# Mrhs121/distributed

Measured on AMD Instinct MI355X. Metric: images/sec (whole node) MNIST CNN at 1/2/4/8 MI355X; DP scaling efficiency, higher is better.
Workload: dtype bf16; 1 GPU; model=MNIST CNN (Conv2D32-3x3-relu, MaxPool2, Dense64-relu, Dense10; 347,146 params), global_batch=64, per_gpu_batch=64, parallelism=dp1, engine=fused_convnet, optimizer=SGD(lr=1e-3), fp32 master weights

## Files before the change

### csrc/bindings.cpp

```cpp
#include <pybind11/pybind11.h>
#include <pybind11/stl.h>

#include <stdexcept>
#include <string>
#include <unordered_map>
#include <vector>

#include "comm.h"
#include "convnet.h"
#include "damd_common.h"
#include "kernels_api.h"
#include "peer_comm.h"
#include "step_executor.h"

namespace py = pybind11;
using namespace damd;

#define HIP_CHECK(x)                                                                    \
  do {                                                                                  \
    hipError_t e_ = (x);                                                                \
    if (e_ != hipSuccess)                                                               \
      throw std::runtime_error(std::string("HIP error: ") + hipGetErrorString(e_) +     \
                               " at " #x);                                              \
  } while (0)

template <typename T>
static T* P_(uintptr_t p) { return reinterpret_cast<T*>(p); }

class ConvNetTrainer : public StepExecutor {
 public:
  ConvNetTrainer(int device, py::dict bufs, int B, int PP, int grad_allreduce)
      : StepExecutor(device), B_(B), PP_(PP), grad_allreduce_(grad_allreduce) {
    if (B <= 0) throw std::invalid_argument("batch must be > 0");
    if (B > 65535) throw std::invalid_argument("per-rank batch must be < 65536 (packed kernel argument)");
    if (PP < 1 || PP > 4) throw std::invalid_argument("positions per slice must be in [1,4]");
    auto g = [&](const char* k) -> uintptr_t { return bufs[k].cast<uintptr_t>(); };
    b_.X = nullptr; b_.labels = nullptr; b_.x_u8 = 0;
    b_.P = P_<float>(g("params")); b_.G = P_<float>(g("grads")); b_.V = P_<float>(g("velocity"));
    b_.ctrl = P_<Ctrl>(g("ctrl"));
    b_.pooled = P_<uint16_t>(g("pooled")); b_.code = P_<uint8_t>(g("code"));
    b_.W1alt = P_<float>(g("w1alt")); b_.V1alt = P_<float>(g("v1alt")); b_.w1bf = P_<uint16_t>(g("w1bf"));
    b_.stamps = bufs.contains("stamps") ? P_<unsigned long long>(g("stamps")) : nullptr;
    b_.eager_w1 = bufs.contains("eager_w1") ? (int)g("eager_w1") : 0;
    b_.hacc = P_<long long>(g("hacc"));
    b_.hconv = P_<long long>(g("hconv"));
    b_.calt = P_<float>(g("calt"));
    b_.ppb = bufs.contains("ppb") ? (int)g("ppb") : PP;
    b_.force_generic = bufs.contains("specialised") ? !(int)g("specialised") : 0;
    b_.xnext = bufs.contains("xnext") ? P_<void>(g("xnext")) : nullptr;
    b_.xtag = bufs.contains("xtag") ? P_<long long>(g("xtag")) : nullptr;
    b_.xcur = bufs.contains("xcur") ? P_<void>(g("xcur")) : nullptr;
    b_.ycur = bufs.contains("ycur") ? P_<int>(g("ycur")) : nullptr;
    if ((b_.xnext == nullptr) != (b_.xtag == nullptr) || (b_.xcur == nullptr) != (b_.ycur == nullptr))
      throw std::invalid_argument("xnext / xtag and xcur / ycur go in pairs");
    const char* ph = getenv("DAMD_PAR_HINT");
    hint_ = !(ph && ph[0] == '0');
    b_.par_hint = -1;
    if (b_.ppb < 1 || b_.ppb > 4) throw std::invalid_argument("bwd positions per slice must be in [1,4]");
    HIP_CHECK(convnet2_set_lds_limits());
  }
  std::vector<std::vector<float>> phase_times(int k) {
    if (!b_.X) throw std::runtime_error("ConvNetTrainer: set_data() not called");
    hipEvent_t ev[4];
    for (auto& e : ev) HIP_CHECK(hipEventCreate(&e));
    std::vector<std::vector<float>> out;
    for (int i = 0; i < k; ++i) {
      HIP_CHECK(hipEventRecord(ev[0], stream_));
      b_.par_hint = hint_ ? par_ : -1;
      HIP_CHECK(convnet2_launch_fwd(b_, B_, PP_, stream_));
      HIP_CHECK(hipEventRecord(ev[1], stream_));
      HIP_CHECK(convnet2_launch_bwd(b_, B_, PP_, stream_));
      par_ ^= 1;
      HIP_CHECK(hipEventRecord(ev[2], stream_));
      if (grad_allreduce_ && !sharded_) {
        if (peer_ && fold_)
          peer_->allreduce_staged((long)convnet_grad_count(PP_), 2 * kConvNetNConv, stream_, b_.hconv);
        else if (peer_) peer_->allreduce(b_.G, (long)convnet_grad_count(PP_), stream_, b_.hconv, 2 * kConvNetNConv);
        else if (comm_) comm_->allreduce_f32_i64(b_.G, convnet_grad_count(PP_), b_.hconv, 2 * kConvNetNConv, stream_);
      }
      HIP_CHECK(hipEventRecord(ev[3], stream_));
      HIP_CHECK(hipEventSynchronize(ev[3]));
      std::vector<float> r(3);
      for (int j = 0; j < 3; ++j) HIP_CHECK(hipEventElapsedTime(&r[j], ev[j], ev[j + 1]));
      out.push_back(r);
    }
    for (auto& e : ev) hipEventDestroy(e);
    return out;
  }
  void set_data(uintptr_t X, uintptr_t labels, int x_u8) {
    b_.X = P_<const void>(X); b_.labels = P_<const int>(labels); b_.x_u8 = x_u8;
    if (b_.xtag) HIP_CHECK(hipMemsetAsync(b_.xtag, 0, sizeof(long long), stream_));
    invalidate_graphs();
  }
  void set_peer_fold(PeerAllreduce* p, bool fold) {
    if (!G_own_) { G_own_ = b_.G; hconv_own_ = b_.hconv; }
    set_peer(p);
    fold_ = fold && p && p->world() > 1;
    if (fold_) {
      const long n = (long)convnet_grad_count(PP_), nfp = (n + 3) / 4 * 4;
      if (PeerAllreduce::message_words(n, 2 * kConvNetNConv) > p->capacity())
        throw std::invalid_argument("peer all-reduce capacity too small for the folded step");
      b_.G = p->in_local();
      b_.hconv = hconv_own_;
      b_.Gr = p->out_local();
      b_.hconv_r = reinterpret_cast<long long*>(p->out_local() + nfp);
    } else {
      b_.G = G_own_; b_.hconv = hconv_own_; b_.Gr = nullptr; b_.hconv_r = nullptr;
    }
    invalidate_graphs();
  }
  bool folded() const { return fold_; }
  void set_sharded(PeerAllreduce* p, uintptr_t hred, int gbf16) {
    if (!p || p->world() < 2 || p->world() > kXMaxRanks) throw std::invalid_argument("sharded step: 2..8 ranks");
    const int NU = 4 * convnet_num_slices(b_.ppb);
    if (p->capacity() < convnet_xin_floats(p->world(), NU) || p->capacity() < convnet_xout_floats(NU))
      throw std::invalid_argument("sharded step: peer staging too small");
    const PeerArgs& a = p->args();
    XArgs x{};
    for (int r = 0; r < p->world(); ++r) {
      if (!a.in[r] || !a.out[r]) throw std::runtime_error("sharded step: peer staging not mapped");
      x.in[r] = a.in[r];
      x.out[r] = a.out[r];
    }
    x.status = a.status;
    x.timeout_ticks = a.timeout_ticks;
    x.world = p->world();
    x.rank = p->rank();
    x.gbf16 = gbf16;
    x.ppb = b_.ppb;
    xa_ = x;
    set_peer(p);
    sharded_ = true;
    fold_ = false;
    HIP_CHECK(hipMemset(p->out_local() + kXFlags, 0,
                        (size_t)(convnet_xout_floats(NU) - kXFlags) * sizeof(float)));
    HIP_CHECK(hipDeviceSynchronize());
    b_.xa = &xa_;
    b_.Gr = p->out_local() + kXGred;
    b_.hconv_r = P_<long long>(hred);
    invalidate_graphs();
  }
  bool sharded() const { return sharded_; }
  void set_exchange_timeout(double s) { xa_.timeout_ticks = (unsigned long long)(s * 1e8); invalidate_graphs(); }
  void gather() {
    if (sharded_) HIP_CHECK(convnet2_launch_gather(b_, PP_, stream_));
  }
  std::vector<float> metric_tail() {
    std::vector<float> t(3);
    gather();
    HIP_CHECK(hipStreamSynchronize(stream_));
    const float* g = b_.Gr ? b_.Gr : b_.G;
    HIP_CHECK(hipMemcpy(t.data(), g + kConvNetNParam, 3 * sizeof(float), hipMemcpyDeviceToHost));
    return t;
  }
  void flush() {
    gather();
    HIP_CHECK(convnet2_launch_flush(b_, B_, stream_));
    par_ = 0;
  }
  int parity() const { return par_; }
  void capture_final(int k) { StepExecutor::capture_final(k); }
  bool run_final(int k) { return StepExecutor::run_final(k); }
  bool warm_final(int k) { return StepExecutor::warm_final(k); }
  int num_slices() const { return convnet_num_slices(PP_); }
  int num_slices_bwd() const { return convnet_num_slices(b_.ppb); }
  int batch() const { return B_; }
  std::string step_kernels() const { return convnet2_specialised(b_, B_, PP_) ? "specialised" : "generic"; }
  int fwd_threads() const { return convnet2_fwd_threads(b_, B_, PP_); }
  int fwd_compiled_threads() const {
    int n = 0;
    HIP_CHECK(convnet2_fwd_compiled_threads(b_, B_, PP_, &n));
    return n;
  }
  int bwd_threads() const { return convnet2_bwd_threads(b_, B_, PP_); }
  int bwd_compiled_threads() const {
    int n = 0;
    HIP_CHECK(convnet2_bwd_compiled_threads(b_, B_, PP_, &n));
    return n;
  }

 protected:
  void enqueue_tail() override { flush(); }
  int phase_value() const override { return par_; }
  void set_phase(int p) override { par_ = p; }
  int phase_after(int p, int k, bool tail) const override { return tail ? 0 : p ^ (k & 1); }
  void enqueue_one_step() override {
    if (!b_.X) throw std::runtime_error("ConvNetTrainer: set_data() not called");
    b_.par_hint = hint_ ? par_ : -1;
    HIP_CHECK(convnet2_launch_step(b_, B_, PP_, stream_));
    par_ ^= 1;
    if (!grad_allreduce_ || sharded_) return;
    long long* aux = b_.hconv;
    const long n64 = 2 * kConvNetNConv;
    if (peer_ && fold_)
      peer_->allreduce_staged((long)convnet_grad_count(PP_), n64, stream_, b_.hconv);
    else if (peer_)
      peer_->allreduce(b_.G, (long)convnet_grad_count(PP_), stream_, aux, n64);
    else if (comm_)
      comm_->allreduce_f32_i64(b_.G, convnet_grad_count(PP_), aux, (size_t)n64, stream_);
  }

 private:
  ConvNetBuffers b_{};
  float* G_own_ = nullptr;
  long long* hconv_own_ = nullptr;
  bool fold_ = false;
  bool sharded_ = false;
  XArgs xa_{};
  int par_ = 0;
  bool hint_ = true;
  int B_, PP_, grad_allreduce_;
};

const char* damd_src_hash();

PYBIND11_MODULE(_C, m) {
  m.doc() = "distributed_amd native runtime (HIP/gfx950 kernels, RCCL, hipGraph executor)";
  m.def("src_hash", []() { return std::string(damd_src_hash()); });
  m.def("graph_nodes", [](uintptr_t gp) {
    hipGraph_t g = reinterpret_cast<hipGraph_t>(gp);
    size_t n = 0;
    HIP_CHECK(hipGraphGetNodes(g, nullptr, &n));
    std::vector<hipGraphNode_t> nodes(n);
    if (n) HIP_CHECK(hipGraphGetNodes(g, nodes.data(), &n));
    std::unordered_map<hipGraphNode_t, int> idx;
    for (size_t i = 0; i < n; ++i) idx[nodes[i]] = (int)i;
    py::list out;
    for (size_t i = 0; i < n; ++i) {
      hipGraphNodeType t;
      HIP_CHECK(hipGraphNodeGetType(nodes[i], &t));
      std::string name;
      if (t == hipGraphNodeTypeKernel) {
        hipKernelNodeParams kp{};
        if (hipGraphKernelNodeGetParams(nodes[i], &kp) == hipSuccess && kp.func) {
          const char* nm = hipKernelNameRefByPtr(kp.func, nullptr);
          if (nm) name = nm;
        }
        (void)hipGetLastError();
      }
      size_t nd = 0;
      HIP_CHECK(hipGraphNodeGetDependencies(nodes[i], nullptr, &nd));
      std::vector<hipGraphNode_t> deps(nd);
      if (nd) HIP_CHECK(hipGraphNodeGetDependencies(nodes[i], deps.data(), &nd));
      std::vector<int> di;
      for (auto d : deps) di.push_back(idx.count(d) ? idx[d] : -1);
      out.append(py::make_tuple((int)t, name, di));
    }
    return out;
  });
  m.attr("CONVNET_NPARAM") = kConvNetNParam;
  m.attr("CONVNET_NGRAD") = kConvNetNGrad;
  m.attr("CONVNET_NCONV") = kConvNetNConv;
  m.def("convnet2_lds_bytes", [](int PP) { return py::make_tuple(convnet2_fwd_lds(PP, 4), convnet2_bwd_lds(PP)); });
  m.def("convnet2_bwd_flag_lds_bytes", [](int PP) { return convnet2_bwd_lds(PP, true); });
  m.def("convnet_num_slices", &convnet_num_slices);
  m.def("convnet_hacc_elems", &convnet_hacc_elems);
  m.def("convnet_grad_count", &convnet_grad_count);

  m.def("device_count", []() { int n = 0; if (hipGetDeviceCount(&n) != hipSuccess) n = 0; return n; });
  m.def("rccl_unique_id", []() { return py::bytes(rccl_unique_id()); });
  m.def("rccl_version", []() { int v = 0; ncclGetVersion(&v); return v; });

  py::class_<RcclComm>(m, "RcclComm")
      .def(py::init([](int n, int r, py::bytes uid, int dev) {
             return new RcclComm(n, r, std::string(uid), dev);
           }),
           py::arg("nranks"), py::arg("rank"), py::arg("uid"), py::arg("device"),
           py::call_guard<py::gil_scoped_release>())
      .def_property_readonly("nranks", &RcclComm::nranks)
      .def_property_readonly("rank", &RcclComm::rank)
      .def_property_readonly("comm_count", &RcclComm::comm_count)
      .def("allreduce",
           [](RcclComm& c, uintptr_t s, uintptr_t r, size_t n, int dt, int op, uintptr_t st) {
             c.allreduce(P_<void>(s), P_<void>(r), n, dt, op, P_<ihipStream_t>(st));
           })
      .def("broadcast",
           [](RcclComm& c, uintptr_t b, size_t n, int dt, int root, uintptr_t st) {
             c.broadcast(P_<void>(b), n, dt, root, P_<ihipStream_t>(st));
           })
      .def("allgather",
           [](RcclComm& c, uintptr_t s, uintptr_t r, size_t n, int dt, uintptr_t st) {
             c.allgather(P_<const void>(s), P_<void>(r), n, dt, P_<ihipStream_t>(st));
           })
      .def("reduce_scatter",
           [](RcclComm& c, uintptr_t s, uintptr_t r, size_t n, int dt, int op, uintptr_t st) {
             c.reduce_scatter(P_<const void>(s), P_<void>(r), n, dt, op, P_<ihipStream_t>(st));
           })
      .def("allreduce_f32_i64",
           [](RcclComm& c, uintptr_t d, size_t n, uintptr_t a, size_t n64, uintptr_t st) {
             c.allreduce_f32_i64(P_<float>(d), n, P_<long long>(a), n64, P_<ihipStream_t>(st));
           })
      .def("abort", &RcclComm::abort)
      .def_property_readonly("aborted", &RcclComm::aborted);

  m.def("stream_wait", [](uintptr_t st, double timeout_s) {
    py::gil_scoped_release nogil;
    return stream_wait_with_deadline(P_<ihipStream_t>(st), timeout_s, nullptr);
  });

  py::class_<PeerAllreduce>(m, "PeerAllreduce")
      .def(py::init<int, int, int, long, int, double>(), py::arg("world"), py::arg("rank"), py::arg("device"),
           py::arg("capacity"), py::arg("blocks") = 64, py::arg("timeout_s") = 120.0)
      .def("handles", [](PeerAllreduce& p) { return py::bytes(p.handles()); })
      .def("open",
           [](PeerAllreduce& p, std::vector<py::bytes> hs) {
             std::vector<std::string> v;
             for (auto& h : hs) v.emplace_back(std::string(h));
             p.open(v);
           })
      .def("allreduce",
           [](PeerAllreduce& p, uintptr_t data, long n, uintptr_t st, uintptr_t aux64, long n64) {
             p.allreduce(P_<float>(data), n, P_<ihipStream_t>(st), P_<long long>(aux64), n64);
           },
           py::arg("data"), py::arg("n"), py::arg("stream"), py::arg("aux64") = 0, py::arg("n64") = 0)
      .def_static("message_words", &PeerAllreduce::message_words)
      .def("link_local", &PeerAllreduce::link_local)
      .def("status", &PeerAllreduce::status)
      .def("clear_status", &PeerAllreduce::clear_status)
      .def("set_timeout", &PeerAllreduce::set_timeout)
      .def_property_readonly("ready", &PeerAllreduce::ready)
      .def_property_readonly("capacity", &PeerAllreduce::capacity)
      .def("peek_out",
           [](PeerAllreduce& p, long off, long n) {
             std::vector<uint32_t> v((size_t)n);
             HIP_CHECK(hipDeviceSynchronize());
             HIP_CHECK(hipMemcpy(v.data(), p.out_local() + off, (size_t)n * 4, hipMemcpyDeviceToHost));
             return v;
           })
      .def_property_readonly("world", &PeerAllreduce::world)
      .def_property_readonly("rank", &PeerAllreduce::rank);

  py::class_<ConvNetTrainer>(m, "ConvNetTrainer")
      .def(py::init<int, py::dict, int, int, int>(), py::arg("device"), py::arg("buffers"),
           py::arg("batch"), py::arg("positions_per_slice") = 4, py::arg("grad_allreduce") = 1)
      .def("set_data", &ConvNetTrainer::set_data, py::arg("x"), py::arg("labels"), py::arg("x_u8") = 0)
      .def("set_comm", [](ConvNetTrainer& t, RcclComm* c) { t.set_comm(c); },
           py::keep_alive<1, 2>())
      .def("set_peer", [](ConvNetTrainer& t, PeerAllreduce* p, bool fold) { t.set_peer_fold(p, fold); },
           py::arg("peer"), py::arg("fold") = false, py::keep_alive<1, 2>())
      .def_property_readonly("folded", &ConvNetTrainer::folded)
      .def("set_sharded", &ConvNetTrainer::set_sharded, py::arg("peer"), py::arg("hred"), py::arg("gbf16") = 0,
           py::keep_alive<1, 2>())
      .def_property_readonly("sharded", &ConvNetTrainer::sharded)
      .def("set_exchange_timeout", &ConvNetTrainer::set_exchange_timeout)
      .def("gather", &ConvNetTrainer::gather)
      .def("restrict_cus", &ConvNetTrainer::restrict_cus, py::arg("part"), py::arg("nparts"))
      .def("metric_tail", &ConvNetTrainer::metric_tail)
      .def("step", &ConvNetTrainer::step, py::call_guard<py::gil_scoped_release>())
      .def("capture", &ConvNetTrainer::capture)
      .def("step_graph_nodes", &ConvNetTrainer::step_graph_nodes, py::arg("steps"))
      .def("run", &ConvNetTrainer::run, py::call_guard<py::gil_scoped_release>())
      .def("capture_final", &ConvNetTrainer::capture_final, py::arg("steps"))
      .def("run_final", &ConvNetTrainer::run_final, py::arg("steps"), py::call_guard<py::gil_scoped_release>())
      .def("warm_final", &ConvNetTrainer::warm_final, py::arg("steps"), py::call_guard<py::gil_scoped_release>())
      .def("phase_times", &ConvNetTrainer::phase_times, py::arg("steps"), py::call_guard<py::gil_scoped_release>())
      .def("flush", &ConvNetTrainer::flush)
      .def("sync", &ConvNetTrainer::sync, py::arg("timeout_s") = 0.0,
           py::call_guard<py::gil_scoped_release>())
      .def("invalidate_graphs", &ConvNetTrainer::invalidate_graphs)
      .def_property_readonly("num_graphs", &ConvNetTrainer::num_graphs)
      .def_property_readonly("num_slices", &ConvNetTrainer::num_slices)
      .def_property_readonly("num_slices_bwd", &ConvNetTrainer::num_slices_bwd)
      .def_property_readonly("batch", &ConvNetTrainer::batch)
      .def_property_readonly("step_kernels", &ConvNetTrainer::step_kernels)
      .def_property_readonly("fwd_threads", &ConvNetTrainer::fwd_threads)
      .def_property_readonly("fwd_compiled_threads", &ConvNetTrainer::fwd_compiled_threads)
      .def_property_readonly("bwd_threads", &ConvNetTrainer::bwd_threads)
      .def_property_readonly("bwd_compiled_threads", &ConvNetTrainer::bwd_compiled_threads)
      .def_property_readonly("parity", &ConvNetTrainer::parity)
      .def_property_readonly("stream", [](ConvNetTrainer& t) { return reinterpret_cast<uintptr_t>(t.stream()); });

  register_kernel_ops(m);
}
```

### csrc/include/convnet.h

```cpp
#pragma once
#include <hip/hip_runtime.h>
#include <stdint.h>

namespace damd {
struct Ctrl;

constexpr int kXMaxRanks = 8;
constexpr int kXPSlot = 2048;
constexpr int kXSmsg = 1408;
constexpr long kXGred = 0;
constexpr long kXSmall = 347648;
constexpr long kXFlags = kXSmall + 2L * kXMaxRanks * kXSmsg;
constexpr int kXPFlagPitch = 2 * kXMaxRanks;
struct XArgs {
  float* in[kXMaxRanks];
  float* out[kXMaxRanks];
  unsigned* status;
  unsigned long long timeout_ticks;
  int world, rank;
  int gbf16;
  int ppb;
};
constexpr long kXG16 = kXFlags + 16384;
inline long convnet_xout_floats(int nunits) { return kXG16 + 5408L * 64 / 2; }
inline long convnet_xin_floats(int world, int nunits) { return (long)world * nunits * kXPSlot; }
struct ConvNetBuffers {
  const void* X; const int* labels;
  int x_u8;
  float* P; float* G; float* V; Ctrl* ctrl;
  float* W1alt; float* V1alt; uint16_t* w1bf;
  uint16_t* pooled ; uint8_t* code ;
  unsigned long long* stamps;
  long long* hacc;
  long long* hconv;
  float* calt;
  int eager_w1;
  float* Gr;
  long long* hconv_r;
  const XArgs* xa;
  void* xnext;
  long long* xtag;
  void* xcur;
  int* ycur;
  int par_hint;
  int ppb;
  int force_generic;
};
constexpr int kConvNetNConv = 320;
constexpr int kConvNetNParam = 347146;
constexpr int kConvNetNGrad = 347152;
int convnet_num_slices(int PP);
long convnet_hacc_elems(int B);
int convnet_f1_lg(int B);
size_t convnet2_fwd_lds(int PP, int lg);
size_t convnet2_bwd_lds(int PP, bool flagship = false);
hipError_t convnet2_launch_step(const ConvNetBuffers& b, int B, int PP, hipStream_t st);
hipError_t convnet2_launch_fwd(const ConvNetBuffers& b, int B, int PP, hipStream_t st);
hipError_t convnet2_launch_bwd(const ConvNetBuffers& b, int B, int PP, hipStream_t st);
hipError_t convnet2_launch_flush(const ConvNetBuffers& b, int B, hipStream_t st);
hipError_t convnet2_launch_gather(const ConvNetBuffers& b, int PP, hipStream_t st);
hipError_t convnet2_set_lds_limits();
bool convnet2_specialised(const ConvNetBuffers& b, int B, int PP);
int convnet2_fwd_threads(const ConvNetBuffers& b, int B, int PP);
hipError_t convnet2_fwd_compiled_threads(const ConvNetBuffers& b, int B, int PP, int* out);
int convnet2_bwd_threads(const ConvNetBuffers& b, int B, int PP);
hipError_t convnet2_bwd_compiled_threads(const ConvNetBuffers& b, int B, int PP, int* out);
size_t convnet_grad_count(int PP);
}
```

### csrc/kernels/convnet_step2.hip

```cpp
#include "convnet_dev.h"

#ifndef DAMD_PROBE_HACC
#define DAMD_PROBE_HACC 0
#endif
#ifndef DAMD_PROBE_HCONV
#define DAMD_PROBE_HCONV 0
#endif

namespace damd {
namespace convnet2 {
using namespace convnet;

constexpr int NAUX2 = NSMALL + 3;
constexpr int HPITCH = HID + 1;
constexpr int ZP = 17;
constexpr int HEAD_FLOATS = CH * HPITCH + 716 + CH * ZP + 2 * CH + 16 * HID + CH;
constexpr int HEAD_BYTES = HEAD_FLOATS * 4;

constexpr int SM_CONV = 0, SM_GRAD = 2 * NCONV, SM_MET = SM_GRAD + NSMALL;
static_assert(SM_MET + 3 <= kXSmsg, "small message");
__device__ __forceinline__ unsigned* x_flags(float* out) { return reinterpret_cast<unsigned*>(out + kXFlags); }
__device__ __forceinline__ unsigned* x_pflag(float* out, int u, int slot) {
  return x_flags(out) + u * kXPFlagPitch + slot;
}
__device__ __forceinline__ unsigned* x_gflag(float* out, int nu, int u, int half) {
  return x_flags(out) + nu * kXPFlagPitch + u * 2 + half;
}
__device__ __forceinline__ unsigned* x_sflag(float* out, int nu, int par, int src) {
  return x_flags(out) + nu * (kXPFlagPitch + 2) + par * kXMaxRanks + src;
}
__device__ __forceinline__ float* x_small(float* out, int par, int src) {
  return out + kXSmall + ((long)par * kXMaxRanks + src) * kXSmsg;
}
__device__ __forceinline__ void x_signal(unsigned* f, unsigned e) {
  __hip_atomic_store(f, e, __ATOMIC_RELAXED, __HIP_MEMORY_SCOPE_SYSTEM);
}
__device__ __forceinline__ void x_wait(const XArgs& xa, unsigned* f, unsigned e, unsigned bit) {
  const unsigned long long t0 = __builtin_amdgcn_s_memrealtime();
  while (__hip_atomic_load(f, __ATOMIC_RELAXED, __HIP_MEMORY_SCOPE_SYSTEM) < e) {
    __builtin_amdgcn_s_sleep(1);
    const unsigned long long dt = __builtin_amdgcn_s_memrealtime() - t0;
    if (dt > xa.timeout_ticks) {
      __hip_atomic_fetch_or(xa.status, bit, __ATOMIC_RELAXED, __HIP_MEMORY_SCOPE_AGENT);
      break;
    }
    if (dt > 100000ull && __hip_atomic_load(xa.status, __ATOMIC_RELAXED, __HIP_MEMORY_SCOPE_AGENT) != 0u) break;
  }
}
constexpr unsigned XW_SMALL = 1u << 8, XW_UNIT = 1u << 9, XW_PART = 1u << 10;
__device__ __forceinline__ uint2 pack_bf16x4(const f32x4& v) {
  return make_uint2((uint32_t)f2bf(v[0]) | ((uint32_t)f2bf(v[1]) << 16),
                    (uint32_t)f2bf(v[2]) | ((uint32_t)f2bf(v[3]) << 16));
}
__device__ __forceinline__ float4 unpack_bf16x4(uint2 q) {
  return make_float4(bf2f((uint16_t)(q.x & 0xffffu)), bf2f((uint16_t)(q.x >> 16)), bf2f((uint16_t)(q.y & 0xffffu)),
                     bf2f((uint16_t)(q.y >> 16)));
}

#ifndef DAMD_FWD_BAL
#define DAMD_FWD_BAL 1
#endif
#ifndef DAMD_FWD_STORES
#define DAMD_FWD_STORES 1
#endif
#ifndef DAMD_FWD_D1REG
#define DAMD_FWD_D1REG 1
#endif
#ifndef DAMD_BWD_NT
#define DAMD_BWD_NT 1024
#endif
#ifndef DAMD_BWD_AUX
#define DAMD_BWD_AUX 1
#endif
struct CfgGeneric {
  static constexpr int PP = 0, LG = 0;
  static constexpr bool B64 = false, EAGER = false, SH = true;
  static constexpr int NT = 512, BAL = 0, STORES = 0;
  static constexpr bool D1REG = false;
  static constexpr int AUX = 0;
};
struct CfgFlagFwd {
  static constexpr int PP = 3, LG = 4;
  static constexpr bool B64 = true, EAGER = true, SH = false;
  static constexpr int BAL = DAMD_FWD_BAL, STORES = DAMD_FWD_STORES, NT = BAL == 1 ? 768 : 512;
  static constexpr bool D1REG = DAMD_FWD_D1REG != 0;
  static_assert(BAL >= 0 && BAL <= 2 && STORES >= 0 && STORES <= 2, "fwd wave mapping");
};
struct CfgFlagBwd {
  static constexpr int PP = 2, LG = 0;
  static constexpr bool B64 = true, EAGER = true, SH = false;
  static constexpr int NT = DAMD_BWD_NT, AUX = DAMD_BWD_AUX;
  static_assert((NT == 512 || NT == 1024) && AUX >= 0 && AUX <= 1, "bwd wave mapping");
};
__host__ __device__ constexpr int aux_split(int NS) {
  const int chunk_aux = (NAUX2 + NS - 1) / NS;
  int ltpe = 0;
  while (ltpe < 6 && (2 << ltpe) * chunk_aux <= 512) ++ltpe;
  return chunk_aux | (ltpe << 16);
}

template <bool U8, class C>
__device__ __forceinline__ void fwd_body(const void* __restrict__ xnext, uint16_t* __restrict__ w1bf,
                                         float* __restrict__ P, float* __restrict__ V,
                                         float* __restrict__ calt, const long long* __restrict__ hconv_r,
                                         const float* __restrict__ G, int bpp, int lge, Ctrl* __restrict__ ctrl,
                                         const void* __restrict__ X, float* __restrict__ W1alt,
                                         float* __restrict__ V1alt, uint16_t* __restrict__ pooled,
                                         uint8_t* __restrict__ code, long long* __restrict__ hacc,
                                         long long* __restrict__ hconv, unsigned long long* st, const XArgs& xa,
                                         const long long* __restrict__ xtag, const int* __restrict__ labels,
                                         void* __restrict__ xcur, int* __restrict__ ycur, int phint) {
  constexpr bool SPEC = C::PP > 0;
  static_assert(!SPEC || (C::B64 && C::EAGER && !C::SH && C::LG == 4), "the one constant configuration");
  constexpr int NT = C::NT, NW = NT / 64, NBQ = SPEC ? (C::PP * 32 * HID / 8 + NT - 1) / NT : 2;
  static_assert(NT % 64 == 0 && NT >= 512 && (SPEC || NT == 512), "row staging and the deferred update map 512 threads");
  static_assert(SPEC || (C::BAL == 0 && C::STORES == 0 && !C::D1REG), "the generic kernels keep the plain mapping");
  const int B = SPEC ? CH : bpp & 0xffff, PP = SPEC ? C::PP : bpp >> 16, lg = SPEC ? C::LG : lge & 0xff;
  const int eager = SPEC ? 1 : lge >> 8;
  extern __shared__ __attribute__((aligned(16))) char smem[];
  const int s = blockIdx.x, tid = threadIdx.x, wave = __builtin_amdgcn_readfirstlane(tid >> 6), lane = tid & 63;
  const bool sh = C::SH && xa.world > 1;
  constexpr int hprobe = DAMD_PROBE_HACC;
  constexpr int NSC = SPEC ? (NPOS + C::PP - 1) / C::PP : 0, IGC = SPEC ? CH >> C::LG : 0;
  const int gx = SPEC ? NSC : (int)gridDim.x;
  const int nblk = SPEC ? NSC * IGC : (int)(gridDim.x * gridDim.y), lin = blockIdx.y * gx + s;
  Stamps sts;
  stamp(sts, st, 0);
  const int IB = 1 << lg, img0 = blockIdx.y * IB;
  const int BP = (B + CH - 1) / CH * CH;
  const int p0 = s * PP, p1 = min(NPOS, p0 + PP), np = p1 - p0, K = np * 32;
  const int KP = kpitch(PP);
  const int npl = SPEC ? PP : np, KC = npl * 32;
  float* xs = reinterpret_cast<float*>(smem);
  uint16_t* as = reinterpret_cast<uint16_t*>(smem + IB * XR * IMG * 4);
  uint16_t* w1t = as + IB * KP;
  uint16_t* wf = w1t + HID * KP;
  float* cb = reinterpret_cast<float*>(wf + WF_BYTES / 2);
  static_assert(NT >= NCONV + 5 * NF, "threads past the conv parameters zero the pad slots");
  const int n4 = K * HID / 4;
  const int r0 = 2 * (p0 / PO);
  const int nrows = 2 * ((p1 - 1) / PO) + 4 - r0;
  XStage<U8> xst;
  long long xt = 0;
  const int xslot = NT > 512 && tid >= 512 ? -1 : tid;
  if (xnext != nullptr) {
    x_load<U8>(xst, xnext, img0, B, SPEC ? IB : B - img0, lg, r0, nrows, xslot);
    xt = *xtag;
  }
  uint4 bq[NBQ];
  if (eager) {
#pragma unroll
    for (int u = 0; u < NBQ; ++u) {
      bq[u] = make_uint4(0u, 0u, 0u, 0u);
      if (tid + u * NT < n4 / 2) bq[u] = reinterpret_cast<const uint4*>(w1bf + p0 * 32 * HID)[tid + u * NT];
    }
  }
  const int tcl = min(tid, NCONV - 1);
  const float cp0 = P[tcl], cp1 = calt[tcl], cv0 = V[tcl], cv1 = calt[NCONV + tcl];
  const long long cq0 = sh ? 0 : hconv_r[NCONV + tcl], cq1 = sh ? 0 : hconv_r[tcl];
  const int si = (lin - (nblk - 2)) * NT + tid;
  const bool small_on = lin >= nblk - 2 && si >= 0 && si < NSMALL;
  const int sic = OFF_B1 + max(0, min(si, NSMALL - 1));
  const float sp = P[sic], sg0 = sh ? 0.f : G[sic], sv = V[sic];
  int wfs[3];
  conv_w_slots(wfs, tid);
  __builtin_amdgcn_sched_barrier(0);

  const Ctrl c = *ctrl;
  const int par = phint >= 0 ? phint : c.wpar;
  if (phint >= 0 && phint != c.wpar && lin == 0 && tid == 0)
    __hip_atomic_fetch_or(&ctrl->bad, 2, __ATOMIC_RELAXED, __HIP_MEMORY_SCOPE_AGENT);
  const unsigned xe = (unsigned)c.xcnt;
  if (lin == 0 && tid == 0) {
    ctrl->cur2 = c.cursor;
    ctrl->par2 = par;
    ctrl->xcnt2 = c.xcnt;
    ctrl->pend2 = c.pending;
  }
  const bool pend = c.pending != 0;
  const long row_base = (long)c.cursor * c.global_batch + c.row0 + img0;
  const bool mom = c.momentum != 0.f;

  const bool xhit = xnext != nullptr && xt == (((long long)c.xgen << 32) | (long long)(unsigned)(c.cursor + 1));
  if (!xhit) x_load<U8>(xst, X, row_base, c.nsamples, SPEC ? IB : B - img0, lg, r0, nrows, xslot);
  constexpr int UPI = U8 ? NPIX / 16 : NPIX / 4;
  const int xcu = lin * NT + tid;
  const bool xcp = xcur != nullptr && xcu < B * UPI;
  uint4 xcv = make_uint4(0u, 0u, 0u, 0u);
  int ycv = -1;
  {
    const long rb0 = (long)c.cursor * c.global_batch + c.row0;
    if (xcp) {
      const int b = xcu / UPI, q = xcu - b * UPI;
      if (xhit) xcv = reinterpret_cast<const uint4*>(xnext)[xcu];
      else if (rb0 + b < c.nsamples)
        xcv = reinterpret_cast<const uint4*>(static_cast<const char*>(X) +
                                             __umul24((unsigned)(rb0 + b), U8 ? NPIX : 4 * NPIX))[q];
    }
    if (xcur != nullptr && lin == 0 && tid < B && rb0 + tid < c.nsamples) ycv = labels[rb0 + tid];
  }
  float4 wv[4], gv[4], vv[4];
  const float* Wcur = par ? W1alt : P + OFF_W1;
  const float* Vcur = par ? V1alt : V + OFF_W1;
  float* Wnext = par ? P + OFF_W1 : W1alt;
  float* Vnext = par ? V + OFF_W1 : V1alt;
  const float4* P4 = reinterpret_cast<const float4*>(Wcur + p0 * 32 * HID);
  const float4* G4 = reinterpret_cast<const float4*>(G + OFF_W1 + p0 * 32 * HID);
  const float4* V4 = reinterpret_cast<const float4*>((mom ? Vcur : Wcur) + p0 * 32 * HID);
  const bool owner = blockIdx.y == 0;
  float4* Wn4 = reinterpret_cast<float4*>(Wnext + p0 * 32 * HID);
  float4* Vn4 = reinterpret_cast<float4*>(Vnext + p0 * 32 * HID);
  uint2* Wb = reinterpret_cast<uint2*>(w1bf + p0 * 32 * HID);
  if (!eager) {
#pragma unroll
    for (int u = 0; u < 4; ++u) {
      const int ic = min(tid + u * 512, n4 - 1);
      wv[u] = P4[ic];
      gv[u] = sh ? make_float4(0.f, 0.f, 0.f, 0.f) : G4[ic];
      vv[u] = V4[ic];
    }
  }
  __builtin_amdgcn_sched_barrier(0);
  const float cp = par ? cp1 : cp0, cv = par ? cv1 : cv0;
  long long cq = par ? cq1 : cq0;
  float sg = sg0;
  if (sh && pend) {
    const int ps = xe & 1;
    float* xo = xa.out[xa.rank];
    if (tid < xa.world) x_wait(xa, x_sflag(xo, 4 * ((NPOS + xa.ppb - 1) / xa.ppb), ps, tid), xe, XW_SMALL);
    __syncthreads();
    long long q = 0;
    float g = 0.f;
    for (int r = 0; r < xa.world; ++r) {
      const float* m = x_small(xo, ps, r);
      q += reinterpret_cast<const long long*>(m + SM_CONV)[tcl];
      if (small_on) g += m[SM_GRAD + max(0, min(si, NSMALL - 1))];
    }
    cq = q;
    sg = g;
    if (lin == nblk - 1 && tid < 3) {
      float a = 0.f;
      for (int r = 0; r < xa.world; ++r) a += x_small(xo, ps, r)[SM_MET + tid];
      float* accp = tid == 0 ? &ctrl->acc_loss : (tid == 1 ? &ctrl->acc_correct : &ctrl->acc_count);
      *accp = (tid == 0 ? c.acc_loss : (tid == 1 ? c.acc_correct : c.acc_count)) + a;
    }
  }

  if (eager) {
#pragma unroll
    for (int u = 0; u < NBQ; ++u) {
      const int i = tid + u * NT;
      if (i < (SPEC ? PP * 32 * HID / 8 : n4 / 2)) {
        const int e = i * 8, kr = e >> 6, n = e & 63;
        const uint32_t w[4] = {bq[u].x, bq[u].y, bq[u].z, bq[u].w};
#pragma unroll
        for (int q = 0; q < 4; ++q) {
          w1t[(n + 2 * q) * KP + kr] = (uint16_t)(w[q] & 0xffffu);
          w1t[(n + 2 * q + 1) * KP + kr] = (uint16_t)(w[q] >> 16);
        }
      }
    }
  }
  auto w1_update = [&]() __attribute__((always_inline)) {
#pragma unroll
    for (int u = 0; u < 4; ++u) {
      const int i = tid + u * 512;
      if (!eager && i < n4) {
        float4 wn, vn;
        sgd_or_keep(pend, wv[u].x, gv[u].x, vv[u].x, c, wn.x, vn.x);
        sgd_or_keep(pend, wv[u].y, gv[u].y, vv[u].y, c, wn.y, vn.y);
        sgd_or_keep(pend, wv[u].z, gv[u].z, vv[u].z, c, wn.z, vn.z);
        sgd_or_keep(pend, wv[u].w, gv[u].w, vv[u].w, c, wn.w, vn.w);
        const int e = i * 4, kr = e >> 6, n = e & 63;
        const uint16_t h0 = f2bf(wn.x), h1 = f2bf(wn.y), h2 = f2bf(wn.z), h3 = f2bf(wn.w);
        w1t[(n + 0) * KP + kr] = h0;
        w1t[(n + 1) * KP + kr] = h1;
        w1t[(n + 2) * KP + kr] = h2;
        w1t[(n + 3) * KP + kr] = h3;
        if (owner) {
          Wn4[i] = wn;
          if (mom) Vn4[i] = vn;
          Wb[i] = make_uint2((uint32_t)h0 | ((uint32_t)h1 << 16), (uint32_t)h2 | ((uint32_t)h3 << 16));
        }
      }
    }
  };
  if (!sh) w1_update();
  float cwn = 0.f, cvn = 0.f;
  if (tid < NCONV) {
    sgd_or_keep(pend, cp, from_fix(cq, CINV), cv, c, cwn, cvn);
    if (tid < OFF_BC) conv_w_store(wf, wfs, cwn);
    else cb[tid - OFF_BC] = cwn;
    if (!__builtin_isfinite(cwn)) __hip_atomic_fetch_or(&ctrl->bad, 1, __ATOMIC_RELAXED, __HIP_MEMORY_SCOPE_AGENT);
  }
  if (tid >= NCONV && tid < NCONV + 5 * NF) wf[wfs[0]] = 0;
  if (small_on) {
    float wn, vn;
    sgd_or_keep(pend, sp, sg, sv, c, wn, vn);
    P[sic] = wn;
    if (mom) V[sic] = vn;
    if (!__builtin_isfinite(wn)) __hip_atomic_fetch_or(&ctrl->bad, 1, __ATOMIC_RELAXED, __HIP_MEMORY_SCOPE_AGENT);
  }
  if (lin == 0 && tid < NCONV) {
    (par ? P : calt)[tid] = cwn;
    if (mom) (par ? V : calt + NCONV)[tid] = cvn;
    hconv[par * NCONV + tid] = 0;
  }
  stamp(sts, st, 1);
  x_store<U8>(xst, xs, lg, nrows);
  lds_barrier();
  stamp(sts, st, 2);

  ConvFrag cf;
  conv_setup(cf, wf, cb, lane);
  stamp(sts, st, 5);
  uint8_t* csl = reinterpret_cast<uint8_t*>(cb + NF);
  conv_pool<NW, C::BAL == 2>(cf, xs, p0, npl, r0, lg, wave, lane, [&](int bu, int bl, int plo, int ch, uint16_t hb, uint8_t cd) {
    as[(bu * KP + plo * 32) + (bl * KP + ch)] = SPEC && plo >= np ? (uint16_t)0 : hb;
    csl[(bu * KC + plo * 32) + (bl * KC + ch)] = cd;
  });
  stamp(sts, st, 6);
  lds_barrier();
  stamp(sts, st, 3);
  auto store_out = [&](int t0, int nt) __attribute__((always_inline)) {
    for (int i = t0; i < KC * (IB / 4); i += nt) {
      if (SPEC && i >= K * (IB / 4)) break;
      const int kk = i >> (lg - 2), bo = 4 * (i & ((1 << (lg - 2)) - 1));
      uint16_t v[4];
#pragma unroll
      for (int e = 0; e < 4; ++e) v[e] = as[(bo + e) * KP + kk];
      uint16_t* dst = pooled + (unsigned)((p0 * NF + kk) * BP + img0 + bo);
      if (SPEC || img0 + bo + 3 < B) {
        *reinterpret_cast<uint2*>(dst) = make_uint2((uint32_t)v[0] | ((uint32_t)v[1] << 16),
                                                   (uint32_t)v[2] | ((uint32_t)v[3] << 16));
      } else {
#pragma unroll
        for (int e = 0; e < 4; ++e)
          if (img0 + bo + e < B) dst[e] = v[e];
      }
    }
    for (int i = t0; i < IB * (KC / 4); i += nt) {
      const int i8 = i >> 3, bo = npl == 3 ? (int)(((unsigned)i8 * 21846u) >> 16) : i8 >> (npl >> 1), w = i - bo * (KC / 4);
      if ((SPEC || img0 + bo < B) && (!SPEC || 4 * w < K))
        *reinterpret_cast<uint32_t*>(code + (unsigned)((img0 + bo) * FEAT + p0 * NF + 4 * w)) =
            reinterpret_cast<const uint32_t*>(csl + bo * KC)[w];
    }
    stamp(sts, st, 7);
  };
  if (C::STORES == 0) store_out(tid, NT);
  if (sh) {
    if (pend) {
      const int sb0 = p0 / xa.ppb, nunits = 4 * ((p1 - 1) / xa.ppb - sb0 + 1), NUb = 4 * ((NPOS + xa.ppb - 1) / xa.ppb);
      if (tid < 2 * nunits) x_wait(xa, x_gflag(xa.out[xa.rank], NUb, 4 * sb0 + (tid >> 1), tid & 1), xe, XW_UNIT);
      __syncthreads();
      if (xa.gbf16) {
        const uint2* R2 = reinterpret_cast<const uint2*>(xa.out[xa.rank] + kXG16) + p0 * 32 * HID / 4;
#pragma unroll
        for (int u = 0; u < 4; ++u) gv[u] = unpack_bf16x4(R2[min(tid + u * 512, n4 - 1)]);
      } else {
        const float4* R4 = reinterpret_cast<const float4*>(xa.out[xa.rank] + kXGred + OFF_W1 + p0 * 32 * HID);
#pragma unroll
        for (int u = 0; u < 4; ++u) gv[u] = R4[min(tid + u * 512, n4 - 1)];
      }
    }
    w1_update();
    lds_barrier();
  }
  const int ko = 8 * (lane >> 4);
  const int ntiles = (IB >> 4) * 4;
  float* part = xs;
  long long* hp = hacc + (long)par * B * HACC_PITCH;
  const int TD1 = ntiles * 64;
  static_assert(!(C::D1REG || C::STORES == 1) || ((1 << C::LG) >> 4) * 4 < NW, "dense-1 tiles: one per wave, waves to spare");
  if constexpr (C::D1REG) {
    if (wave < ntiles) {
      const int mt = wave >> 2, nt = wave & 3;
      f32x4 acc = {0.f, 0.f, 0.f, 0.f};
      const int ar = 16 * mt + (lane & 15), bn = 16 * nt + (lane & 15);
      for (int ks = 0; ks < npl; ++ks) {
        const bf16x8 a = ld_frag(as + ar * KP + ks * 32 + ko);
        const bf16x8 bb = ld_frag(w1t + bn * KP + ks * 32 + ko);
        acc = mfma16(a, bb, acc);
      }
      stamp(sts, st, 8);
#pragma unroll
      for (int j = 0; j < (hprobe == 1 ? 0 : hprobe == 2 ? 2 : 4); ++j) {
        const int r = 16 * mt + 4 * (lane >> 4) + j;
        atomic_add_i64(hp + (unsigned)((img0 + r) * HACC_PITCH + bn), to_fix(acc[j], HSCALE, &ctrl->bad));
      }
    } else {
      if (C::STORES == 1) store_out(tid - TD1, NT - TD1);
      stamp(sts, st, 8);
    }
    stamp(sts, st, 9);
  } else {
    for (int t = wave; t < ntiles; t += NW) {
      const int mt = t >> 2, nt = t & 3;
      f32x4 acc = {0.f, 0.f, 0.f, 0.f};
      const int ar = 16 * mt + (lane & 15), bn = 16 * nt + (lane & 15);
      for (int ks = 0; ks < npl; ++ks) {
        const bf16x8 a = ld_frag(as + ar * KP + ks * 32 + ko);
        const bf16x8 bb = ld_frag(w1t + bn * KP + ks * 32 + ko);
        acc = mfma16(a, bb, acc);
      }
#pragma unroll
      for (int j = 0; j < 4; ++j) part[(16 * mt + 4 * (lane >> 4) + j) * HID + bn] = acc[j];
    }
    if (C::STORES == 1 && wave >= ntiles) store_out(tid - TD1, NT - TD1);
    stamp(sts, st, 8);
    lds_barrier();
    stamp(sts, st, 9);
    for (int r = wave; r < (hprobe == 1 ? 0 : hprobe == 2 ? IB / 2 : IB); r += NW)
      if (SPEC || img0 + r < B) atomic_add_i64(hp + (unsigned)((img0 + r) * HACC_PITCH + lane), to_fix(part[r * HID + lane], HSCALE, &ctrl->bad));
  }
  if (C::STORES == 2) store_out(tid, NT);
  if (xcp) reinterpret_cast<uint4*>(xcur)[xcu] = xcv;
  if (xcur != nullptr && lin == 0 && tid < B) ycur[tid] = ycv;
  stamp(sts, st, 4);
  if (st != nullptr && lin < 256) {
    if (tid == 0)
      for (int i = 0; i < 10; ++i) st[lin * 16 + i] = C::STORES == 1 && i == 7 ? 0ull : sts.t[i];
    const int wsel = lin % NW;
    if (tid == 64 * wsel) {
      st[lin * 16 + 10] = sts.t[5];
      st[lin * 16 + 11] = sts.t[6];
      st[lin * 16 + 12] = sts.t[8];
      st[lin * 16 + 13] = sts.t[4];
      st[lin * 16 + 14] = (unsigned long long)(wsel | (NW << 8));
    }
  }
}

template <bool U8>
__global__ __launch_bounds__(512) void fwd(const void* __restrict__ xnext, uint16_t* __restrict__ w1bf,
                                           float* __restrict__ P, float* __restrict__ V,
                                           float* __restrict__ calt, const long long* __restrict__ hconv_r,
                                           const float* __restrict__ G, int bpp, int lge, Ctrl* __restrict__ ctrl,
                                           const void* __restrict__ X, float* __restrict__ W1alt,
                                           float* __restrict__ V1alt, uint16_t* __restrict__ pooled,
                                           uint8_t* __restrict__ code, long long* __restrict__ hacc,
                                           long long* __restrict__ hconv, unsigned long long* st, const XArgs xa,
                                           const long long* __restrict__ xtag, const int* __restrict__ labels,
                                           void* __restrict__ xcur, int* __restrict__ ycur, int phint) {
  fwd_body<U8, CfgGeneric>(xnext, w1bf, P, V, calt, hconv_r, G, bpp, lge, ctrl, X, W1alt, V1alt, pooled, code, hacc,
                           hconv, st, xa, xtag, labels, xcur, ycur, phint);
}

template <bool U8>
__global__ __launch_bounds__(CfgFlagFwd::NT) void fwd_flag(const void* __restrict__ xnext,
                                                const long long* __restrict__ xtag,
                                                uint16_t* __restrict__ w1bf, float* __restrict__ P,
                                                float* __restrict__ V, float* __restrict__ calt,
                                                const long long* __restrict__ hconv_r, const float* __restrict__ G,
                                                Ctrl* __restrict__ ctrl, const void* __restrict__ X,
                                                uint16_t* __restrict__ pooled, uint8_t* __restrict__ code,
                                                long long* __restrict__ hacc, long long* __restrict__ hconv,
                                                unsigned long long* st, const int* __restrict__ labels,
                                                void* __restrict__ xcur, int* __restrict__ ycur, int phint) {
  fwd_body<U8, CfgFlagFwd>(xnext, w1bf, P, V, calt, hconv_r, G, 0, 0, ctrl, X, nullptr, nullptr, pooled, code, hacc,
                           hconv, st, XArgs{}, xtag, labels, xcur, ycur, phint);
}

__device__ __forceinline__ void exchange_tail(const XArgs& xa, Ctrl* ctrl, const float* G, const long long* hconv_p,
                                              const f32x4* accw, unsigned xe, int s, int NS, int np, int p0, int dn,
                                              int dm0, int lane, int tid, bool xown, int xo, int xu) {
  __shared__ int last_flag;
  const int NU = 4 * NS, W = xa.world, ps = xe & 1;
  damd_publish_drain();
  DAMD_PUBLISH_WAVE();
  if (!xown && lane == 0) x_signal(x_pflag(xa.out[xo], xu, xa.rank * 2 + dm0), xe);
  __syncthreads();
  if (tid == 0) {
    __builtin_amdgcn_fence(__ATOMIC_RELEASE, "agent");
    const int t = __hip_atomic_fetch_add(&ctrl->ticket, 1, __ATOMIC_RELAXED, __HIP_MEMORY_SCOPE_AGENT);
    const int last = (t % NS) == NS - 1;
    if (last) __builtin_amdgcn_fence(__ATOMIC_ACQUIRE, "agent");
    last_flag = last;
  }
  __syncthreads();
  if (last_flag) {
    const float* hc = reinterpret_cast<const float*>(hconv_p);
    for (int i = tid; i < SM_MET + 3; i += 512) {
      const float v = i < SM_GRAD ? hc[i] : (i < SM_MET ? G[OFF_B1 + i - SM_GRAD] : G[OFF_LOSS + i - SM_MET]);
      for (int r = 0; r < W; ++r) x_small(xa.out[r], ps, xa.rank)[i] = v;
    }
    damd_publish_drain();
    __syncthreads();
    DAMD_PUBLISH_WG();
    if (tid < W) x_signal(x_sflag(xa.out[tid], NU, ps, xa.rank), xe);
  }
  if (xown) {
    if (lane < W && lane != xa.rank) x_wait(xa, x_pflag(xa.out[xa.rank], xu, lane * 2 + dm0), xe, XW_PART);
    asm volatile("" ::: "memory");
    f32x4 g[MAXPP];
#pragma unroll
    for (int i = 0; i < MAXPP; ++i) g[i] = f32x4{0.f, 0.f, 0.f, 0.f};
    for (int r = 0; r < W; ++r) {
      const float* slot = xa.in[xa.rank] + ((long)r * NU + xu) * kXPSlot;
#pragma unroll
      for (int i = 0; i < MAXPP; ++i) {
        if (i >= np) break;
        float4 v;
        if (xa.gbf16)
          v = unpack_bf16x4(r == xa.rank ? pack_bf16x4(accw[i])
                                         : reinterpret_cast<const uint2*>(slot)[(dm0 * MAXPP + i) * 64 + lane]);
        else
          v = r == xa.rank ? make_float4(accw[i][0], accw[i][1], accw[i][2], accw[i][3])
                           : reinterpret_cast<const float4*>(slot)[(dm0 * MAXPP + i) * 64 + lane];
        g[i][0] += v.x;
        g[i][1] += v.y;
        g[i][2] += v.z;
        g[i][3] += v.w;
      }
    }
    const int lr16 = lane & 15;
    if (xa.gbf16) {
      for (int r = 0; r < W; ++r) {
        uint32_t* dst = reinterpret_cast<uint32_t*>(xa.out[r] + kXG16) + ((long)p0 * 32 * HID + 16 * dn + lr16) / 2;
#pragma unroll
        for (int i = 0; i < MAXPP; ++i) {
          if (i >= np) break;
          const int mt = dm0 + 2 * i;
#pragma unroll
          for (int j = 0; j < 4; ++j) {
            const uint32_t h = f2bf(g[i][j]);
            const uint32_t o = (uint32_t)__shfl_xor((int)h, 1);
            if (!(lr16 & 1)) dst[(16 * mt + 4 * (lane >> 4) + j) * (HID / 2)] = h | (o << 16);
          }
        }
      }
    } else {
      for (int r = 0; r < W; ++r) {
        float* dst = xa.out[r] + kXGred + OFF_W1 + (long)p0 * 32 * HID + 16 * dn + lr16;
#pragma unroll
        for (int i = 0; i < MAXPP; ++i) {
          if (i >= np) break;
          const int mt = dm0 + 2 * i;
#pragma unroll
          for (int j = 0; j < 4; ++j) dst[(16 * mt + 4 * (lane >> 4) + j) * HID] = g[i][j];
        }
      }
    }
    damd_publish_drain();
    DAMD_PUBLISH_WAVE();
    if (lane < W) x_signal(x_gflag(xa.out[lane], NU, xu, dm0), xe);
  }
}

template <bool U8, bool ONE, class C>
__device__ __forceinline__ void bwd_body(long long* __restrict__ hacc, const int* __restrict__ ycur,
                                         const void* __restrict__ xcur, int phint, int bpp, const float* P,
                                         const uint16_t* w1bf, const uint16_t* __restrict__ pooled,
                                         const uint8_t* __restrict__ code, Ctrl* __restrict__ ctrl,
                                         const void* __restrict__ X, const int* __restrict__ labels,
                                         float* __restrict__ G, long long* __restrict__ hconv,
                                         int eager_, float* Pw, float* Vw, uint16_t* w1bf_out,
                                         unsigned long long* st, const float* __restrict__ Gr, const XArgs& xa,
                                         void* __restrict__ xnext, long long* __restrict__ xtag, int auxm_) {
  constexpr bool SPEC = C::PP > 0;
  static_assert(!SPEC || (ONE && C::B64 && C::EAGER && !C::SH), "the one constant configuration");
  const int B = SPEC ? CH : bpp & 0xffff, PP = SPEC ? C::PP : bpp >> 16;
  const int eager = SPEC ? 1 : eager_;
  extern __shared__ __attribute__((aligned(16))) char smem[];
  const bool sh = C::SH && xa.world > 1;
  constexpr int cprobe = DAMD_PROBE_HCONV;
  Stamps sts;
  unsigned long long wst_dh = 0, wst_cg = 0;
  stamp(sts, st, 0);
  constexpr int NSC = SPEC ? (NPOS + C::PP - 1) / C::PP : 1;
  const int s = blockIdx.x, tid = threadIdx.x, NS = SPEC ? NSC : (int)gridDim.x;
  const int auxm = SPEC ? aux_split(NSC) : auxm_;
  const int p0 = s * PP, p1 = min(NPOS, p0 + PP), np = p1 - p0, K = np * 32;
  const int KD = PP * 32 + 4;
  const int KC = PP * 32;
  const int npl = SPEC ? PP : np;
  constexpr int NT = C::NT, NW = NT / 64;
  constexpr bool W16 = NT == 1024, AUXD = C::AUX != 0;
  static_assert(SPEC || (NT == 512 && !AUXD), "the generic kernels keep the plain mapping");
  const int RB = AUXD ? HEAD_BYTES + CH * KD * 4 : max(CH * KD * 4, HEAD_BYTES);
  float* xs = reinterpret_cast<float*>(smem);
  float* dps = reinterpret_cast<float*>(smem + XS_BYTES + (AUXD ? HEAD_BYTES : 0));
  uint16_t* pt = reinterpret_cast<uint16_t*>(smem + XS_BYTES + RB);
  uint16_t* dht = pt + PP * 32 * HP;
  uint16_t* dhs = dht + 2 * HID * HP;
  uint16_t* w1s = dhs + 2 * CH * HP;
  uint8_t* cs = reinterpret_cast<uint8_t*>(w1s + PP * 32 * HP);
  float* red = reinterpret_cast<float*>(pt);
  float* hs = reinterpret_cast<float*>(smem + XS_BYTES);
  float* spl = hs + CH * HPITCH;
  float* zs = spl + 716;
  float* rl = zs + CH * ZP;
  float* rc = rl + CH;
  float* db1p = rc + CH;
  int* ylds = reinterpret_cast<int*>(db1p + 16 * HID);
  const int r0 = 2 * (p0 / PO);
  const int nrows = 2 * ((p1 - 1) / PO) + 4 - r0;
  const int wave = tid >> 6, lane = tid & 63;
  const int ko = 8 * (lane >> 4), lr16 = lane & 15;

  const int chunk_aux = auxm & 0xffff, ltpe = auxm >> 16, tpe = 1 << ltpe;
  const int ae_local = tid >> ltpe, aq = tid & (tpe - 1);
  const int ae = s * chunk_aux + ae_local;
  const bool aux_on = ae_local < chunk_aux && ae < NAUX2;
  const int aec = min(ae, NAUX2 - 1);
  float arsum = 0.f;

  const float ag_old = sh ? 0.f : Gr[OFF_LOSS + max(0, min(aec - NSMALL, 2))];
  float spv0 = 0.f, spv1 = 0.f;
  if (!W16 || tid < NSMALL) spv0 = P[OFF_B1 + tid];
  if (!W16 && tid + 512 < NSMALL) spv1 = P[OFF_B1 + tid + 512];
  constexpr int HQS = W16 ? 4 : 3, HQN = W16 ? 2 : 4;
  uint4 hq0, hq1, hq2, hq3;
  const bool hq_early = ONE && phint >= 0;
  auto load_hq = [&](int chunk, int p) __attribute__((always_inline)) {
    const int r = tid >> HQS, q = tid & ((1 << HQS) - 1);
    const int row = min(chunk * CH + r, B - 1);
    const uint4* hp = reinterpret_cast<const uint4*>(hacc + (unsigned)((p * B + row) * HACC_PITCH + q * 2 * HQN));
    hq0 = hp[0];
    hq1 = hp[1];
    if (HQN > 2) {
      hq2 = hp[2];
      hq3 = hp[3];
    } else {
      hq2 = hq3 = make_uint4(0u, 0u, 0u, 0u);
    }
  };
  if (hq_early) load_hq(0, phint);
  const int n8 = K * HID / 8;
  uint4 wv0, wv1;
  constexpr int WS = W16 ? 256 : 512;
  const int wt = W16 ? tid - 768 : tid;
  wv0 = wv1 = make_uint4(0u, 0u, 0u, 0u);
  if (wt >= 0 && wt < n8) wv0 = reinterpret_cast<const uint4*>(w1bf + p0 * 32 * HID)[wt];
  if ((!SPEC || WS < PP * 32 * HID / 8) && wt >= 0 && wt + WS < n8)
    wv1 = reinterpret_cast<const uint4*>(w1bf + p0 * 32 * HID)[wt + WS];
  constexpr int NB = W16 ? 512 : ONE ? 256 : 512;
  const int bt = ONE ? tid - 256 : tid;
  const bool bw = !ONE || (bt >= 0 && bt < NB);
  const int ct = W16 ? tid - 768 : bt;
  const bool cw = W16 ? ct >= 0 : bw;
  XStage<U8> xst, xst1;
  uint4 pv0, pv1, pv2, pv3;
  uint4 cv, cv1;
  bool cok = false, cok1 = false;
  int ylab = 0;
  bool yval = false;
  const int BP = (B + CH - 1) / CH * CH;
  const int kc = K / 16;
  constexpr int NPV = SPEC ? (C::PP * 32 * 8 + NB - 1) / NB : 4, KCM = SPEC ? 2 * C::PP : 1;
  auto div_kc = [&](int i) __attribute__((always_inline)) {
    return np == 3 ? (int)(((unsigned)(i >> 1) * 21846u) >> 16) : (i >> 1) >> (np >> 1);
  };
  static_assert(MAXPP == 4, "div_kc covers np = 1..4");
  auto load_pv = [&](uint4& v, int i, int chunk) __attribute__((always_inline)) {
    v = make_uint4(0u, 0u, 0u, 0u);
    if (i < K * 8) v = *reinterpret_cast<const uint4*>(pooled + (__umul24(p0 * NF + (i >> 3), BP) + chunk * CH + (i & 7) * 8));
  };
  auto load_cv = [&](uint4& v, bool& ok, int i, int chunk) __attribute__((always_inline)) {
    if constexpr (SPEC) {
      const int bb = i / KCM, q = i - bb * KCM;
      ok = i < CH * KCM && q < kc;
      v = make_uint4(0u, 0u, 0u, 0u);
      if (ok) v = *reinterpret_cast<const uint4*>(code + (__umul24(bb, FEAT) + p0 * NF + q * 16));
      return;
    }
    const int bb = div_kc(i), q = i - bb * kc, lb = chunk * CH + bb;
    ok = i < CH * kc && lb < B;
    v = make_uint4(0u, 0u, 0u, 0u);
    if (i < CH * kc) v = *reinterpret_cast<const uint4*>(code + (__umul24(min(lb, B - 1), FEAT) + p0 * NF + q * 16));
  };
  auto load_indep = [&](int chunk) __attribute__((always_inline)) {
    if (bw) {
      load_pv(pv0, bt, chunk);
      if (NPV > 1) load_pv(pv1, bt + NB, chunk);
      if (ONE && NPV > 2) {
        load_pv(pv2, bt + 2 * NB, chunk);
        load_pv(pv3, bt + 3 * NB, chunk);
      }
    }
    if (cw) {
      load_cv(cv, cok, ct, chunk);
      if (ONE && !W16 && (!SPEC || NB < CH * KCM)) load_cv(cv1, cok1, ct + NB, chunk);
    }
    if (ycur != nullptr) {
      const int b = chunk * CH + min(tid, CH - 1);
      ylab = ycur[min(b, B - 1)];
      yval = tid < CH && b < B && ylab >= 0;
      if (bw) {
        x_load<U8>(xst, xcur, chunk * CH, B, B - chunk * CH, LG_CH, r0, nrows, bt);
        if (ONE && !W16) x_load<U8>(xst1, xcur, chunk * CH, B, B - chunk * CH, LG_CH, r0, nrows, bt + NB);
      }
    }
  };
  load_indep(0);
  __builtin_amdgcn_sched_barrier(0);

  const Ctrl c = *ctrl;
  const int cur = c.cur2, par = phint >= 0 ? phint : c.par2;
  if (phint >= 0 && phint != c.par2 && s == 0 && tid == 0)
    __hip_atomic_fetch_or(&ctrl->bad, 2, __ATOMIC_RELAXED, __HIP_MEMORY_SCOPE_AGENT);
  const unsigned xe = (unsigned)c.xcnt2 + 1u;
  if (s == 0 && tid == 0) {
    ctrl->cursor = next_cursor(c, cur);
    ctrl->iterations = c.iterations + 1;
    ctrl->wpar = c.wpar ^ 1;
    ctrl->pending = 1;
    if (sh) ctrl->xcnt = (int)xe;
  }
  const long gstart = (long)cur * c.global_batch;
  const long row_base = gstart + c.row0;
  const int gcount = (int)min((long)c.global_batch, (long)c.nsamples - gstart);
  const float inv = gcount > 0 ? 1.f / (float)gcount : 0.f;
  const int ncur = next_cursor(c, cur);
  constexpr int UPI = U8 ? NPIX / 16 : NPIX / 4;
  const int xpu = s * 512 + tid;
  const bool xpf = ONE && xnext != nullptr && (!W16 || tid < 512) && xpu < B * UPI;
  uint4 xnv = make_uint4(0u, 0u, 0u, 0u);

  auto load_dep = [&](int chunk) __attribute__((always_inline)) {
    if (!hq_early || chunk > 0) load_hq(chunk, par);
    if (ycur == nullptr) {
      {
        const int b = chunk * CH + min(tid, CH - 1);
        const long g = row_base + b;
        yval = tid < CH && b < B && g < c.nsamples;
        ylab = labels[max(0L, min(g, (long)c.nsamples - 1))];
      }
      if (bw) {
        x_load<U8>(xst, X, row_base + chunk * CH, c.nsamples, B - chunk * CH, LG_CH, r0, nrows, bt);
        if (ONE && !W16) x_load<U8>(xst1, X, row_base + chunk * CH, c.nsamples, B - chunk * CH, LG_CH, r0, nrows, bt + NB);
      }
    }
  };
  auto load_chunk = [&](int chunk) __attribute__((always_inline)) {
    load_indep(chunk);
    load_dep(chunk);
  };
  auto store_head = [&]() __attribute__((always_inline)) {
    if (!W16 || tid < NSMALL) spl[tid] = spv0;
    if (!W16 && tid + 512 < NSMALL) spl[tid + 512] = spv1;
    if (tid < CH) ylds[tid] = yval ? ylab : -1;
  };
  auto store_pv = [&](const uint4& v, int i) __attribute__((always_inline)) {
    if (i < (SPEC ? PP * 32 * 8 : K * 8)) *reinterpret_cast<uint4*>(pt + (i >> 3) * HP + (i & 7) * 8) = v;
  };
  auto store_cv = [&](const uint4& v, bool ok, int i) __attribute__((always_inline)) {
    if constexpr (SPEC) {
      const int bb = i / KCM, q = i - bb * KCM;
      if (i < CH * KCM) *reinterpret_cast<uint4*>(cs + bb * KC + q * 16) = ok ? v : make_uint4(0u, 0u, 0u, 0u);
      return;
    }
    if (i < CH * kc) {
      const int bb = div_kc(i), q = i - bb * kc;
      *reinterpret_cast<uint4*>(cs + bb * KC + q * 16) = ok ? v : make_uint4(0u, 0u, 0u, 0u);
    }
  };
  auto store_body = [&]() __attribute__((always_inline)) {
    if (cw) {
      store_cv(cv, cok, ct);
      if (ONE && !W16 && (!SPEC || NB < CH * KCM)) store_cv(cv1, cok1, ct + NB);
    }
    if (!bw) return;
    store_pv(pv0, bt);
    if (NPV > 1) store_pv(pv1, bt + NB);
    if (ONE && NPV > 2) {
      store_pv(pv2, bt + 2 * NB);
      store_pv(pv3, bt + 3 * NB);
    }
    x_store<U8>(xst, xs, LG_CH, nrows);
    if (ONE && !W16) x_store<U8>(xst1, xs, LG_CH, nrows);
  };
  auto store_chunk = [&](int chunk) __attribute__((always_inline)) {
    store_body();
    store_head();
  };
  load_dep(0);
  if (xpf) {
    const int b = xpu / UPI, q = xpu - b * UPI;
    const int g = (int)((long)ncur * c.global_batch + c.row0) + b;
    if (g < c.nsamples)
      xnv = reinterpret_cast<const uint4*>(static_cast<const char*>(X) + __umul24((unsigned)g, U8 ? NPIX : 4 * NPIX))[q];
  }
  const int n8s = SPEC ? PP * 32 * HID / 8 : n8;
  if (wt >= 0 && wt < n8s) *reinterpret_cast<uint4*>(w1s + (wt >> 3) * HP + (wt & 7) * 8) = wv0;
  if (wt >= 0 && wt + WS < n8s) *reinterpret_cast<uint4*>(w1s + ((wt + WS) >> 3) * HP + (wt & 7) * 8) = wv1;

  constexpr int TPW = W16 ? 1 : MAXPP;
  const int dn = wave & 3, dm0 = wave >> 2;
  const bool mom = c.momentum != 0.f;
  float ew[ONE ? MAXPP : 1][4], ev[ONE ? MAXPP : 1][4];
  f32x4 accw[MAXPP];
#pragma unroll
  for (int i = 0; i < MAXPP; ++i) accw[i] = f32x4{0.f, 0.f, 0.f, 0.f};
  const int NU = 4 * NS, xu = 4 * s + dn;
  const int xo = !sh ? 0 : (xa.world & (xa.world - 1)) == 0 ? xu & (xa.world - 1) : xu % xa.world;
  const bool xown = sh && xo == xa.rank;
  auto push_partials = [&]() __attribute__((always_inline)) {
    if (!sh || xown) return;
    float* slot = xa.in[xo] + ((long)xa.rank * NU + xu) * kXPSlot;
    if (xa.gbf16) {
      uint2* dst = reinterpret_cast<uint2*>(slot) + dm0 * MAXPP * 64 + lane;
#pragma unroll
      for (int i = 0; i < MAXPP; ++i)
        if (i < np) dst[i * 64] = pack_bf16x4(accw[i]);
    } else {
      float4* dst = reinterpret_cast<float4*>(slot) + dm0 * MAXPP * 64 + lane;
#pragma unroll
      for (int i = 0; i < MAXPP; ++i)
        if (i < np) dst[i * 64] = make_float4(accw[i][0], accw[i][1], accw[i][2], accw[i][3]);
    }
  };
  const int ch = tid & 31, grp = (tid >> 5) & 15, half = tid >> 9;
  float gw[9], gb = 0.f;
#pragma unroll
  for (int t = 0; t < 9; ++t) gw[t] = 0.f;
  auto aux_sums = [&]() __attribute__((always_inline)) {
    if (!aux_on) return;
    float a = 0.f;
    if (aec < HID) {
      if (aq == 0)
#pragma unroll
        for (int q = 0; q < 16; ++q) a += db1p[q * HID + aec];
    } else if (aec < HID + HID * NCLS) {
      const int kk = (aec - HID) / NCLS, cc = aec - HID - kk * NCLS;
      for (int r = aq; r < CH; r += tpe) a = fmaf(hs[r * HPITCH + kk], zs[r * ZP + cc], a);
    } else if (aec < NSMALL) {
      const int cc = aec - HID - HID * NCLS;
      for (int r = aq; r < CH; r += tpe) a += zs[r * ZP + cc];
    } else if (aec < NSMALL + 2) {
      const float* src = aec == NSMALL ? rl : rc;
      for (int r = aq; r < CH; r += tpe) a += src[r];
    }
    arsum += a;
  };
  const int nchunks = ONE ? 1 : (B + CH - 1) / CH;

  for (int chunk = 0; chunk < nchunks; ++chunk) {
    if (chunk) {
      lds_barrier();
      load_chunk(chunk);
    }
    if (ONE) store_head();
    else store_chunk(chunk);
    lds_barrier();
    stamp(sts, st, 1);
    if (ONE && eager) {
#pragma unroll
      for (int i = 0; i < TPW; ++i) {
        const int mt = W16 ? dm0 : dm0 + 2 * i, pi = W16 ? dm0 >> 1 : i;
        if (pi >= npl) break;
        if (SPEC && pi >= np) continue;
        const unsigned e0 = OFF_W1 + (unsigned)((p0 * 32 + 16 * mt + 4 * (lane >> 4)) * HID + 16 * dn + lr16);
        const float* pw = Pw + e0;
        const float* vw = Vw + e0;
#pragma unroll
        for (int j = 0; j < 4; ++j) {
          ew[i][j] = pw[j * HID];
          ev[i][j] = mom ? vw[j * HID] : 0.f;
        }
      }
    }
    {
      const int r = tid >> HQS, q = tid & ((1 << HQS) - 1);
      const bool rv = chunk * CH + r < B;
      const uint4 hq[4] = {hq0, hq1, hq2, hq3};
#pragma unroll
      for (int u = 0; u < HQN; ++u) {
        const long long a = (long long)(((unsigned long long)hq[u].y << 32) | hq[u].x);
        const long long b = (long long)(((unsigned long long)hq[u].w << 32) | hq[u].z);
        const int n = q * 2 * HQN + 2 * u;
        hs[r * HPITCH + n] = rv ? fmaxf(from_fix(a, HINV) + spl[n], 0.f) : 0.f;
        hs[r * HPITCH + n + 1] = rv ? fmaxf(from_fix(b, HINV) + spl[n + 1], 0.f) : 0.f;
      }
    }
    lds_barrier();
    stamp(sts, st, 6);
    if (ONE && wave >= 4) {
      store_body();
      stamp(sts, st, 12);
    }
    if (wave < 4) {
      const int mt = wave, lr = lane & 15, kq = lane >> 4;
      float av[HID / 4], bv[HID / 4];
#pragma unroll
      for (int ks = 0; ks < HID / 4; ++ks) {
        const int k = 4 * ks + kq;
        av[ks] = hs[(16 * mt + lr) * HPITCH + k];
        bv[ks] = spl[HID + k * NCLS + min(lr, NCLS - 1)];
      }
      int yv4[4];
#pragma unroll
      for (int j = 0; j < 4; ++j) yv4[j] = ylds[16 * mt + 4 * kq + j];
      f32x4 acc = {0.f, 0.f, 0.f, 0.f};
      if (ONE) stamp(sts, st, 9);
#pragma unroll
      for (int ks = 0; ks < HID / 4; ++ks) acc = mfma4(av[ks], lr < NCLS ? bv[ks] : 0.f, acc);
      const float b2v = lr < NCLS ? spl[HID + HID * NCLS + lr] : 0.f;
      float v[4], m[4], e[4], lse[4];
      int am[4];
#pragma unroll
      for (int j = 0; j < 4; ++j) v[j] = lr < NCLS ? acc[j] + b2v : -INFINITY;
#pragma unroll
      for (int j = 0; j < 4; ++j) m[j] = row16_max(v[j]);
#pragma unroll
      for (int j = 0; j < 4; ++j) e[j] = lr < NCLS ? __expf(v[j] - m[j]) : 0.f;
#pragma unroll
      for (int j = 0; j < 4; ++j) e[j] = row16_sum(e[j]);
      if (ONE) stamp(sts, st, 10);
#pragma unroll
      for (int j = 0; j < 4; ++j) {
        lse[j] = m[j] + __builtin_amdgcn_logf(e[j]) * 0.693147180559945f;
        am[j] = row16_min(v[j] == m[j] ? lr : 16);
      }
      if (ONE) stamp(sts, st, 11);
#pragma unroll
      for (int j = 0; j < 4; ++j) {
        const int r = 16 * mt + 4 * kq + j;
        const int yv = yv4[j];
        const bool valid = yv >= 0;
        const int y = valid ? yv : 0;
        zs[r * ZP + lr] = valid ? (__expf(v[j] - lse[j]) - (lr == y ? 1.f : 0.f)) * inv : 0.f;
        if (lr == y) {
          rl[r] = valid ? (lse[j] - v[j]) : 0.f;
          rc[r] = (valid && am[j] == y) ? 1.f : 0.f;
        }
      }
    }
    if (ONE && wave < 4) stamp(sts, st, 12);
    lds_barrier();
    stamp(sts, st, 7);
    constexpr int NDH = 16 / NW;
    float za[NDH][3], wb[NDH][3], hm[NDH][4];
#pragma unroll
    for (int ti = 0; ti < NDH; ++ti) {
      const int t = wave + 8 * ti, mt = t >> 2, nt = t & 3, lr = lane & 15, kq = lane >> 4;
#pragma unroll
      for (int ks = 0; ks < 3; ++ks) {
        const int k = 4 * ks + kq;
        za[ti][ks] = k < NCLS ? zs[(16 * mt + lr) * ZP + k] : 0.f;
        wb[ti][ks] = k < NCLS ? spl[HID + (16 * nt + lr) * NCLS + k] : 0.f;
      }
#pragma unroll
      for (int j = 0; j < 4; ++j) hm[ti][j] = hs[(16 * mt + 4 * kq + j) * HPITCH + 16 * nt + lr];
    }
#pragma unroll
    for (int ti = 0; ti < NDH; ++ti) {
      const int t = wave + 8 * ti, mt = t >> 2, nt = t & 3, lr = lane & 15, kq = lane >> 4;
      f32x4 acc = {0.f, 0.f, 0.f, 0.f};
#pragma unroll
      for (int ks = 0; ks < 3; ++ks) acc = mfma4(za[ti][ks], wb[ti][ks], acc);
      const int n = 16 * nt + lr, rb = 16 * mt + 4 * kq;
      uint16_t hi[4], lo[4];
      float dsum = 0.f;
#pragma unroll
      for (int j = 0; j < 4; ++j) {
        const float d = hm[ti][j] > 0.f ? acc[j] : 0.f;
        dsum += d;
        hi[j] = f2bf(d);
        lo[j] = bf16_lo(d, hi[j]);
        dhs[(rb + j) * HP + n] = hi[j];
        dhs[CH * HP + (rb + j) * HP + n] = lo[j];
      }
      *reinterpret_cast<uint2*>(dht + n * HP + rb) =
          make_uint2((uint32_t)hi[0] | ((uint32_t)hi[1] << 16), (uint32_t)hi[2] | ((uint32_t)hi[3] << 16));
      *reinterpret_cast<uint2*>(dht + HID * HP + n * HP + rb) =
          make_uint2((uint32_t)lo[0] | ((uint32_t)lo[1] << 16), (uint32_t)lo[2] | ((uint32_t)lo[3] << 16));
      db1p[(4 * mt + kq) * HID + n] = dsum;
    }
    if (st != nullptr) wst_dh = __builtin_amdgcn_s_memrealtime();
    lds_barrier();
    stamp(sts, st, 8);
    if (!AUXD) {
      aux_sums();
      lds_barrier();
    }
    stamp(sts, st, 2);
#pragma unroll
    for (int i = 0; i < TPW; ++i) {
      const int mt = W16 ? dm0 : dm0 + 2 * i;
      if ((W16 ? dm0 >> 1 : i) >= npl) break;
#pragma unroll
      for (int kk = 0; kk < 2; ++kk) {
        const bf16x8 a = ld_frag(pt + (16 * mt + lr16) * HP + kk * 32 + ko);
        const bf16x8 bh = ld_frag(dht + (16 * dn + lr16) * HP + kk * 32 + ko);
        const bf16x8 bl = ld_frag(dht + HID * HP + (16 * dn + lr16) * HP + kk * 32 + ko);
        accw[i] = mfma16(a, bh, accw[i]);
        accw[i] = mfma16(a, bl, accw[i]);
      }
    }
    if (ONE && sh) push_partials();
    if (ONE && eager) {
#pragma unroll
      for (int i = 0; i < TPW; ++i) {
        const int mt = W16 ? dm0 : dm0 + 2 * i, pi = W16 ? dm0 >> 1 : i;
        if (pi >= npl) break;
        if (SPEC && pi >= np) continue;
        const unsigned e0 = OFF_W1 + (unsigned)((p0 * 32 + 16 * mt + 4 * (lane >> 4)) * HID + 16 * dn + lr16);
        float* pw = Pw + e0;
        float* vw = Vw + e0;
        uint16_t* bw = w1bf_out + (e0 - OFF_W1);
#pragma unroll
        for (int j = 0; j < 4; ++j) {
          float wn, vn;
          sgd_update(ew[i][j], accw[i][j], ev[i][j], c.lr, c.momentum, c.nesterov, wn, vn);
          pw[j * HID] = wn;
          if (mom) vw[j * HID] = vn;
          bw[j * HID] = f2bf(wn);
        }
      }
    }
    {
      const int pm = wave & 3;
#pragma unroll
      for (int i = 0; i < TPW; ++i) {
        if (!W16 && i >= npl) break;
        const int nt = W16 ? wave >> 2 : (wave >> 2) + 2 * i;
        f32x4 a4 = {0.f, 0.f, 0.f, 0.f};
#pragma unroll
        for (int kk = 0; kk < 2; ++kk) {
          const bf16x8 ah = ld_frag(dhs + (16 * pm + lr16) * HP + kk * 32 + ko);
          const bf16x8 al = ld_frag(dhs + CH * HP + (16 * pm + lr16) * HP + kk * 32 + ko);
          const bf16x8 bb = ld_frag(w1s + (16 * nt + lr16) * HP + kk * 32 + ko);
          a4 = mfma16(ah, bb, a4);
          a4 = mfma16(al, bb, a4);
        }
#pragma unroll
        for (int j = 0; j < 4; ++j) dps[(16 * pm + 4 * (lane >> 4) + j) * KD + 16 * nt + lr16] = a4[j];
      }
    }
    if (C::AUX == 1) aux_sums();
    if (st != nullptr) wst_cg = __builtin_amdgcn_s_memrealtime();
    lds_barrier();
    stamp(sts, st, 3);
    auto conv_grad = [&](auto t0c, auto t1c) __attribute__((always_inline)) {
      constexpr int T0 = decltype(t0c)::value, T1 = decltype(t1c)::value;
#pragma unroll
      for (int ii = 0; ii < 4; ++ii) {
        const int bb = grp * 4 + ii;
        for (int pl = 0; pl < npl; ++pl) {
          if (SPEC && pl >= np) continue;
          const int cd = cs[bb * KC + pl * 32 + ch];
          const int pos = p0 + pl, py = pos / PO, px = pos - py * PO;
          const float dv0 = dps[bb * KD + pl * 32 + ch];
          const float d = (cd & 4) ? dv0 : 0.f;
          const int y0 = 2 * py + ((cd >> 1) & 1) - r0, x0 = 2 * px + (cd & 1);
          const float* xp = xs + (bb * XR + y0) * IMG + x0;
          float xv[9];
#pragma unroll
          for (int t = T0; t < T1; ++t) xv[t] = xp[(t / 3) * IMG + (t % 3)];
#pragma unroll
          for (int t = T0; t < T1; ++t) gw[t] = fmaf(d, xv[t], gw[t]);
          if (T1 == 9) gb += d;
        }
      }
    };
    using std::integral_constant;
    if (!W16) conv_grad(integral_constant<int, 0>{}, integral_constant<int, 9>{});
    else if (half == 0) conv_grad(integral_constant<int, 0>{}, integral_constant<int, 5>{});
    else conv_grad(integral_constant<int, 5>{}, integral_constant<int, 9>{});
  }
  stamp(sts, st, 4);
  if (!ONE && sh) push_partials();
#pragma unroll
  for (int i = 0; i < MAXPP; ++i) {
    if (i >= np || (ONE && eager) || sh) break;
    const int mt = dm0 + 2 * i;
#pragma unroll
    for (int j = 0; j < 4; ++j) {
      const int k = 16 * mt + 4 * (lane >> 4) + j;
      G[OFF_W1 + (unsigned)((p0 * 32 + k) * HID + 16 * dn + lr16)] = accw[i][j];
    }
  }
  lds_barrier();
#pragma unroll
  for (int t = 0; t < 9; ++t)
    if (!W16 || half == (t >= 5 ? 1 : 0)) red[grp * NCONV + t * NF + ch] = gw[t];
  if (!W16 || half == 1) red[grp * NCONV + OFF_BC + ch] = gb;
  float* ared = dps;
  if (!W16 || tid < 512) ared[tid] = arsum;
  lds_barrier();
  for (int i = tid; i < (cprobe ? 0 : NCONV); i += NT) {
    float a = 0.f;
#pragma unroll
    for (int r = 0; r < 16; ++r) a += red[r * NCONV + i];
    atomic_add_i64(hconv + par * NCONV + i, to_fix(a, CSCALE, &ctrl->bad));
  }
  if (aux_on && aq == 0) {
    float tot = 0.f;
    for (int q = 0; q < tpe; ++q) tot += ared[ae_local * tpe + q];
    if (ae < NSMALL) {
      G[OFF_B1 + ae] = tot;
    } else {
      const int m = ae - NSMALL;
      float* accp = m == 0 ? &ctrl->acc_loss : (m == 1 ? &ctrl->acc_correct : &ctrl->acc_count);
      const float old = m == 0 ? c.acc_loss : (m == 1 ? c.acc_correct : c.acc_count);
      if (!sh) *accp = c.pend2 ? old + ag_old : old;
      G[OFF_LOSS + m] = m == 0 && c.bad ? __builtin_nanf("") : m < 2 ? tot : (float)max(0, min(B, gcount - c.row0));
    }
  }
  {
    long long* hz = hacc + (long)(par ^ 1) * B * HACC_PITCH;
    if (!W16 || tid < 512)
      for (int i = s * 512 + tid; i < B * HID / 2; i += NS * 512)
        *reinterpret_cast<uint4*>(hz + (i >> 5) * HACC_PITCH + (i & 31) * 2) = make_uint4(0u, 0u, 0u, 0u);
  }
  if (xpf) reinterpret_cast<uint4*>(xnext)[xpu] = xnv;
  if (ONE && xnext != nullptr && s == 0 && tid == 0) *xtag = ((long long)c.xgen << 32) | (long long)(unsigned)(ncur + 1);
  if (C::SH && sh) exchange_tail(xa, ctrl, G, hconv + par * NCONV, accw, xe, s, NS, np, p0, dn, dm0, lane, tid, xown, xo, xu);
  stamp(sts, st, 5);
  stamp_flush(sts, st, 13);
  if (st != nullptr && tid == 256) st[blockIdx.x * 16 + 13] = sts.t[12];
  if (st != nullptr && tid == 64 * (s % NW)) {
    st[blockIdx.x * 16 + 14] = (wst_dh & 0x00ffffffffffffffull) | ((unsigned long long)(s % NW) << 56);
    st[blockIdx.x * 16 + 15] = (wst_cg & 0x00ffffffffffffffull) | ((unsigned long long)NW << 56);
  }
}

template <bool U8, bool ONE>
__global__ __launch_bounds__(512) void bwd(long long* __restrict__ hacc, const int* __restrict__ ycur,
                                           const void* __restrict__ xcur, int phint, int bpp, const float* P,
                                           const uint16_t* w1bf, const uint16_t* __restrict__ pooled,
                                           const uint8_t* __restrict__ code, Ctrl* __restrict__ ctrl,
                                           const void* __restrict__ X, const int* __restrict__ labels,
                                           float* __restrict__ G, long long* __restrict__ hconv,
                                           int eager, float* Pw, float* Vw, uint16_t* w1bf_out,
                                           unsigned long long* st, const float* __restrict__ Gr, const XArgs xa,
                                           void* __restrict__ xnext, long long* __restrict__ xtag, int auxm) {
  bwd_body<U8, ONE, CfgGeneric>(hacc, ycur, xcur, phint, bpp, P, w1bf, pooled, code, ctrl, X, labels, G, hconv, eager,
                                Pw, Vw, w1bf_out, st, Gr, xa, xnext, xtag, auxm);
}

template <bool U8>
__global__ __launch_bounds__(CfgFlagBwd::NT) void bwd_flag(long long* __restrict__ hacc, const int* __restrict__ ycur,
                                                const void* __restrict__ xcur, const float* P, const uint16_t* w1bf,
                                                const uint16_t* __restrict__ pooled,
                                                const uint8_t* __restrict__ code, int phint,
                                                const float* __restrict__ Gr, Ctrl* __restrict__ ctrl,
                                                const void* __restrict__ X, const int* __restrict__ labels,
                                                float* __restrict__ G, long long* __restrict__ hconv, float* Pw,
                                                float* Vw, uint16_t* w1bf_out, unsigned long long* st,
                                                void* __restrict__ xnext, long long* __restrict__ xtag) {
  bwd_body<U8, true, CfgFlagBwd>(hacc, ycur, xcur, phint, 0, P, w1bf, pooled, code, ctrl, X, labels, G, hconv, 1, Pw,
                                 Vw, w1bf_out, st, Gr, XArgs{}, xnext, xtag, 0);
}

__global__ __launch_bounds__(1024) void flush(float* __restrict__ P, float* __restrict__ G, float* __restrict__ V,
                                             const float* __restrict__ W1alt, const float* __restrict__ V1alt,
                                             long long* __restrict__ hconv, const float* __restrict__ calt,
                                             long long* __restrict__ hacc, int B, int eager,
                                             uint16_t* __restrict__ w1bf, Ctrl* __restrict__ ctrl,
                                             long long* __restrict__ hconv_w) {
  const Ctrl c = *ctrl;
  const bool mom = c.momentum != 0.f, pend = c.pending != 0;
  const long long* hg = hconv + (c.wpar ^ 1) * NCONV;
  const int nvisit = eager ? NPARAM - (OFF_B1 - OFF_W1) : NPARAM;
  for (int iv = blockIdx.x * blockDim.x + threadIdx.x; iv < nvisit; iv += gridDim.x * blockDim.x) {
    const int i = eager && iv >= OFF_W1 ? iv + (OFF_B1 - OFF_W1) : iv;
    const bool w1 = i >= OFF_W1 && i < OFF_B1;
    const bool alt1 = !eager && c.wpar && w1, altc = c.wpar && i < NCONV;
    const float w = alt1 ? W1alt[i - OFF_W1] : (altc ? calt[i] : P[i]);
    const float v = alt1 ? V1alt[i - OFF_W1] : (altc ? calt[NCONV + i] : V[i]);
    const float g = i < NCONV ? from_fix(hg[i], CINV) : G[i];
    float wn, vn;
    sgd_or_keep(pend && !(eager && w1), w, g, v, c, wn, vn);
    P[i] = wn;
    if (mom) V[i] = vn;
    if (w1) w1bf[i - OFF_W1] = f2bf(wn);
  }
  const int rp = c.wpar ^ 1;
  for (int i = blockIdx.x * blockDim.x + threadIdx.x; i < 2 * NCONV + 2 * B * HID; i += gridDim.x * blockDim.x) {
    if (i < 2 * NCONV) {
      const bool read_parity = i / NCONV == rp;
      if (!read_parity) hconv[i] = 0;
      if (!read_parity || hconv_w != hconv) hconv_w[i] = 0;
    } else {
      const int j = i - 2 * NCONV;
      hacc[(j >> 6) * HACC_PITCH + (j & 63)] = 0;
    }
  }
  if (blockIdx.x == 0 && threadIdx.x == 0 && pend) {
    ctrl->acc_loss = c.acc_loss + G[OFF_LOSS];
    ctrl->acc_correct = c.acc_correct + G[OFF_CORR];
    ctrl->acc_count = c.acc_count + G[OFF_CNT];
    G[OFF_LOSS] = G[OFF_CORR] = G[OFF_CNT] = 0.f;
  }
  __syncthreads();
  if (threadIdx.x == 0) {
    if (gridDim.x == 1 ||
        __hip_atomic_fetch_add(&ctrl->flush_ticket, 1, __ATOMIC_RELAXED, __HIP_MEMORY_SCOPE_AGENT) ==
            (int)gridDim.x - 1) {
      ctrl->wpar = 0;
      ctrl->pending = 0;
      ctrl->flush_ticket = 0;
      ctrl->ticket = 0;
    }
  }
}

__global__ __launch_bounds__(512) void sh_gather(Ctrl* __restrict__ ctrl, const XArgs xa, long long* __restrict__ hred,
                                                 int NS, int PP) {
  const Ctrl c = *ctrl;
  if (!c.pending) return;
  const unsigned xe = (unsigned)c.xcnt;
  const int ps = xe & 1, NU = 4 * NS, tid = threadIdx.x;
  float* xo = xa.out[xa.rank];
  for (int u = blockIdx.x; u < NU; u += gridDim.x) {
    if (tid < 2) x_wait(xa, x_gflag(xo, NU, u, tid), xe, XW_UNIT);
    __syncthreads();
    if (xa.gbf16) {
      const int sl = u >> 2, q = u & 3, k0 = sl * PP * 32, k1 = min(FEAT, k0 + PP * 32);
      const uint16_t* g16 = reinterpret_cast<const uint16_t*>(xo + kXG16);
      for (int e = tid; e < (k1 - k0) * 16; e += 512) {
        const long idx = (long)(k0 + (e >> 4)) * HID + 16 * q + (e & 15);
        xo[kXGred + OFF_W1 + idx] = bf2f(g16[idx]);
      }
    }
  }
  if (blockIdx.x != 0) return;
  if (tid < xa.world) x_wait(xa, x_sflag(xo, NU, ps, tid), xe, XW_SMALL);
  __syncthreads();
  for (int i = tid; i < NSMALL + 3; i += 512) {
    float a = 0.f;
    for (int r = 0; r < xa.world; ++r) a += x_small(xo, ps, r)[SM_GRAD + i];
    xo[kXGred + (i < NSMALL ? OFF_B1 + i : OFF_LOSS + i - NSMALL)] = a;
  }
  for (int i = tid; i < NCONV; i += 512) {
    long long q = 0;
    for (int r = 0; r < xa.world; ++r) q += reinterpret_cast<const long long*>(x_small(xo, ps, r) + SM_CONV)[i];
    hred[(c.wpar ^ 1) * NCONV + i] = q;
  }
}

}

int convnet_num_slices(int PP) { return (convnet::NPOS + PP - 1) / PP; }
long convnet_hacc_elems(int B) { return 2L * B * convnet::HACC_PITCH; }
size_t convnet_grad_count(int) { return (size_t)convnet::NGRAD; }
int convnet_f1_lg(int B) { return B <= 256 ? 4 : 6; }

size_t convnet2_fwd_lds(int PP, int lg) {
  using namespace convnet;
  const int KP = kpitch(PP), IB = 1 << lg;
  const size_t xsb = (size_t)IB * XR * IMG * 4, partb = (size_t)IB * HID * 4;
  return (xsb > partb ? xsb : partb) + (size_t)(IB + HID) * KP * 2 + CONV_LDS_BYTES + (size_t)IB * PP * 32 + 256 * 4;
}
size_t convnet2_bwd_lds(int PP, bool flagship) {
  using namespace convnet;
  const int KD = PP * 32 + 4;
  const size_t dpsb = (size_t)CH * KD * 4;
  const size_t rb = flagship && convnet2::CfgFlagBwd::AUX != 0 ? (size_t)convnet2::HEAD_BYTES + dpsb
                    : dpsb > (size_t)convnet2::HEAD_BYTES     ? dpsb
                                                               : (size_t)convnet2::HEAD_BYTES;
  const size_t redb = (size_t)16 * NCONV * 4;
  const size_t ptdht = (size_t)PP * 32 * HP * 2 + (size_t)2 * HID * HP * 2;
  return XS_BYTES + rb + (ptdht > redb ? ptdht : redb) + (size_t)2 * CH * HP * 2 + (size_t)PP * 32 * HP * 2 +
         (size_t)CH * PP * 32 + 16 + 256 * 4;
}

static int eager2(const ConvNetBuffers& b, int B) { return b.eager_w1 && B <= convnet::CH ? 1 : 0; }

static XArgs xargs(const ConvNetBuffers& b) {
  if (b.xa) return *b.xa;
  XArgs a{};
  return a;
}

static int ppb_of(const ConvNetBuffers& b, int PP) { return b.ppb > 0 ? b.ppb : PP; }

bool convnet2_specialised(const ConvNetBuffers& b, int B, int PP) {
  using namespace convnet;
  using namespace convnet2;
  return !b.force_generic && !b.xa && !b.Gr && !b.hconv_r && B == CH && PP == CfgFlagFwd::PP &&
         convnet_f1_lg(B) == CfgFlagFwd::LG && ppb_of(b, PP) == CfgFlagBwd::PP && eager2(b, B) == 1;
}

template <bool U8>
static void launch2_fwd(const ConvNetBuffers& b, int B, int PP, hipStream_t st) {
  using namespace convnet;
  const int NS = convnet_num_slices(PP);
  const int lg = convnet_f1_lg(B);
  const dim3 g1(NS, (B + (1 << lg) - 1) >> lg);
  if (convnet2_specialised(b, B, PP)) {
    hipLaunchKernelGGL((convnet2::fwd_flag<U8>), g1, dim3(convnet2::CfgFlagFwd::NT), convnet2_fwd_lds(PP, lg), st,
                       b.xnext, b.xtag, b.w1bf, b.P, b.V, b.calt, b.hconv, b.G, b.ctrl, b.X, b.pooled, b.code, b.hacc,
                       b.hconv, b.stamps, b.labels, b.xcur, b.ycur, b.par_hint);
    return;
  }
  hipLaunchKernelGGL((convnet2::fwd<U8>), g1, dim3(512), convnet2_fwd_lds(PP, lg), st,
                     B <= CH ? b.xnext : nullptr, b.w1bf, b.P, b.V, b.calt, b.hconv_r ? b.hconv_r : b.hconv,
                     b.Gr ? b.Gr : b.G, B | (PP << 16), lg | (eager2(b, B) << 8), b.ctrl, b.X, b.W1alt, b.V1alt,
                     b.pooled, b.code, b.hacc, b.hconv, b.stamps, xargs(b), b.xtag, b.labels,
                     B <= CH ? b.xcur : nullptr, b.ycur, b.par_hint);
}

template <bool U8>
static void launch2_bwd(const ConvNetBuffers& b, int B, int PPf, hipStream_t st) {
  using namespace convnet;
  const int PP = ppb_of(b, PPf);
  const int NS = convnet_num_slices(PP);
  const int auxm = convnet2::aux_split(NS);
  if (convnet2_specialised(b, B, PPf))
    hipLaunchKernelGGL((convnet2::bwd_flag<U8>), dim3(NS), dim3(convnet2::CfgFlagBwd::NT), convnet2_bwd_lds(PP, true), st, b.hacc, b.ycur, b.xcur,
                       b.P, b.w1bf, b.pooled, b.code, b.par_hint, b.G, b.ctrl, b.X, b.labels, b.G, b.hconv, b.P, b.V,
                       b.w1bf, b.stamps ? b.stamps + 2 * 256 * 16 : nullptr, b.xnext, b.xtag);
  else if (B <= CH)
    hipLaunchKernelGGL((convnet2::bwd<U8, true>), dim3(NS), dim3(512), convnet2_bwd_lds(PP), st, b.hacc,
                       B <= CH ? b.ycur : nullptr, B <= CH ? b.xcur : nullptr, b.par_hint, B | (PP << 16), b.P,
                       b.w1bf, b.pooled, b.code, b.ctrl, b.X, b.labels, b.G, b.hconv, eager2(b, B), b.P, b.V, b.w1bf,
                       b.stamps ? b.stamps + 2 * 256 * 16 : nullptr, b.Gr ? b.Gr : b.G, xargs(b), b.xnext, b.xtag,
                       auxm);
  else
    hipLaunchKernelGGL((convnet2::bwd<U8, false>), dim3(NS), dim3(512), convnet2_bwd_lds(PP), st, b.hacc,
                       B <= CH ? b.ycur : nullptr, B <= CH ? b.xcur : nullptr, b.par_hint, B | (PP << 16), b.P,
                       b.w1bf, b.pooled, b.code, b.ctrl, b.X, b.labels, b.G, b.hconv, eager2(b, B), b.P, b.V, b.w1bf,
                       b.stamps ? b.stamps + 2 * 256 * 16 : nullptr, b.Gr ? b.Gr : b.G, xargs(b), b.xnext, b.xtag,
                       auxm);
}

int convnet2_fwd_threads(const ConvNetBuffers& b, int B, int PP) {
  return convnet2_specialised(b, B, PP) ? convnet2::CfgFlagFwd::NT : 512;
}

hipError_t convnet2_fwd_compiled_threads(const ConvNetBuffers& b, int B, int PP, int* out) {
  const void* f = convnet2_specialised(b, B, PP)
                      ? (b.x_u8 ? (const void*)convnet2::fwd_flag<true> : (const void*)convnet2::fwd_flag<false>)
                      : (b.x_u8 ? (const void*)convnet2::fwd<true> : (const void*)convnet2::fwd<false>);
  hipFuncAttributes at;
  const hipError_t e = hipFuncGetAttributes(&at, f);
  if (e == hipSuccess) *out = at.maxThreadsPerBlock;
  return e;
}

int convnet2_bwd_threads(const ConvNetBuffers& b, int B, int PP) {
  return convnet2_specialised(b, B, PP) ? convnet2::CfgFlagBwd::NT : 512;
}

hipError_t convnet2_bwd_compiled_threads(const ConvNetBuffers& b, int B, int PP, int* out) {
  const void* f = convnet2_specialised(b, B, PP)
                      ? (b.x_u8 ? (const void*)convnet2::bwd_flag<true> : (const void*)convnet2::bwd_flag<false>)
                  : B <= convnet::CH
                      ? (b.x_u8 ? (const void*)convnet2::bwd<true, true> : (const void*)convnet2::bwd<false, true>)
                      : (b.x_u8 ? (const void*)convnet2::bwd<true, false> : (const void*)convnet2::bwd<false, false>);
  hipFuncAttributes at;
  const hipError_t e = hipFuncGetAttributes(&at, f);
  if (e == hipSuccess) *out = at.maxThreadsPerBlock;
  return e;
}

hipError_t convnet2_launch_fwd(const ConvNetBuffers& b, int B, int PP, hipStream_t st) {
  if (!b.hacc || !b.hconv || !b.calt || B > 0xffff) return hipErrorInvalidValue;
  if (b.x_u8) launch2_fwd<true>(b, B, PP, st);
  else launch2_fwd<false>(b, B, PP, st);
  return hipGetLastError();
}

hipError_t convnet2_launch_bwd(const ConvNetBuffers& b, int B, int PP, hipStream_t st) {
  if (!b.hacc || !b.hconv || !b.calt || B > 0xffff) return hipErrorInvalidValue;
  if (convnet2_bwd_lds(ppb_of(b, PP), convnet2_specialised(b, B, PP)) > 160 * 1024) return hipErrorInvalidValue;
  if (b.xa && b.xa->ppb != ppb_of(b, PP)) return hipErrorInvalidValue;
  if (b.x_u8) launch2_bwd<true>(b, B, PP, st);
  else launch2_bwd<false>(b, B, PP, st);
  return hipGetLastError();
}

hipError_t convnet2_launch_step(const ConvNetBuffers& b, int B, int PP, hipStream_t st) {
  hipError_t e = convnet2_launch_fwd(b, B, PP, st);
  return e != hipSuccess ? e : convnet2_launch_bwd(b, B, PP, st);
}

hipError_t convnet2_launch_gather(const ConvNetBuffers& b, int PP, hipStream_t st) {
  if (!b.xa || b.xa->world < 2 || !b.hconv_r) return hipErrorInvalidValue;
  const int ppb = ppb_of(b, PP);
  hipLaunchKernelGGL(convnet2::sh_gather, dim3(57), dim3(512), 0, st, b.ctrl, *b.xa, b.hconv_r, convnet_num_slices(ppb),
                     ppb);
  return hipGetLastError();
}

hipError_t convnet2_launch_flush(const ConvNetBuffers& b, int B, hipStream_t st) {
  hipLaunchKernelGGL(convnet2::flush, dim3(eager2(b, B) ? 1 : 340), dim3(eager2(b, B) ? 1024 : 256), 0, st, b.P, b.Gr ? b.Gr : b.G, b.V,
                     b.W1alt, b.V1alt, b.hconv_r ? b.hconv_r : b.hconv, b.calt, b.hacc, B, eager2(b, B), b.w1bf, b.ctrl,
                     b.hconv);
  return hipGetLastError();
}

hipError_t convnet2_set_lds_limits() {
  const void* fns[10] = {(const void*)convnet2::fwd<false>,        (const void*)convnet2::fwd<true>,
                         (const void*)convnet2::bwd<false, true>,  (const void*)convnet2::bwd<true, true>,
                         (const void*)convnet2::bwd<false, false>, (const void*)convnet2::bwd<true, false>,
                         (const void*)convnet2::fwd_flag<false>,   (const void*)convnet2::fwd_flag<true>,
                         (const void*)convnet2::bwd_flag<false>,   (const void*)convnet2::bwd_flag<true>};
  for (const void* f : fns) {
    hipFuncAttributes at;
    hipError_t e = hipFuncGetAttributes(&at, f);
    if (e != hipSuccess) return e;
    e = hipFuncSetAttribute(f, hipFuncAttributeMaxDynamicSharedMemorySize, 160 * 1024 - (int)at.sharedSizeBytes);
    if (e != hipSuccess) return e;
  }
  return hipSuccess;
}

}
```

### distributed_amd/engine/fused_convnet.py

```python
from __future__ import annotations

import struct

import numpy as np
import torch

from ..utils import env
from ..utils import logging as dlog
from .base import Engine, ExchangeFault
from .data import DataFeed


class ExchangeSelfTestError(RuntimeError):
    """A pinned device gradient exchange (DAMD_ALLREDUCE=xgmi | sharded) failed its start-up
    self-test (engine/xchg_selftest.py).  Raised on EVERY rank (the outcome is a collective
    vote), so a caller may catch it and go on with another transport consistently."""

NPARAM = 347146
NGRAD = 347152
HID, NCLS, FEAT, NCONV = 64, 10, 5408, 320
(C_LR, C_MOM, C_NEST, C_NS, C_ROW0, C_GB, C_CUR, C_IT, C_CA, C_CB, C_AL, C_AC, C_AN, C_WRAP, C_CUR2, C_CUR3, C_WPAR,
 C_FLUSHT, C_PEND, C_PAR2, C_BAD, C_XCNT, C_XCNT2, C_TICKET, C_PEND2, C_XGEN) = range(26)
SHAPES = [(3, 3, 1, 32), (32,), (5408, 64), (64,), (64, 10), (10,)]


def _xchg_fault_at(rank: int, world: int):
    spec = env.get_str("DAMD_XCHG_FAULT_AT", "")
    if not spec or world < 2:
        return None
    r, _, st = spec.partition(":")
    return int(st) if int(r) == rank else None


def _f2i(f: float) -> int:
    return struct.unpack("<i", struct.pack("<f", float(f)))[0]


def _i2f(i: int) -> float:
    return struct.unpack("<f", struct.pack("<i", int(i)))[0]


class FusedConvNetEngine(Engine):
    name = "fused_convnet"

    @staticmethod
    def eligible(model, strategy):
        from ..keras import layers as L
        from ..keras import losses, optimizers

        if strategy.device.type != "cuda":
            return False, "not on a GPU"
        ls = [l for l in getattr(model, "layers", []) if not isinstance(l, L.InputLayer)]
        if len(ls) != 5:
            return False, "layer count"
        if model._regularized():
            return False, "regularizers"
        if model.optimizer.clipping()[0] is not None:
            return False, "gradient clipping"
        if not isinstance(model.optimizer.learning_rate, (int, float)):
            return False, "learning-rate schedule"
        c, p, f, d1, d2 = ls
        if not (isinstance(c, L.Conv2D) and c.filters == 32 and c.kernel_size == (3, 3) and c.strides == (1, 1)
                and c.padding == "valid" and c.dilation_rate == (1, 1) and c.use_bias
                and c.activation.__name__ == "relu" and tuple(c.input_shape or ())[1:] == (28, 28, 1)):
            return False, "conv layer"
        if not (isinstance(p, L.MaxPooling2D) and p.pool_size == (2, 2) and p.strides == (2, 2)
                and p.padding == "valid"):
            return False, "pool layer"
        if not isinstance(f, L.Flatten):
            return False, "flatten"
        if not (isinstance(d1, L.Dense) and d1.units == 64 and d1.use_bias and d1.activation.__name__ == "relu"):
            return False, "dense"
        if not (isinstance(d2, L.Dense) and d2.units == 10 and d2.use_bias and d2.activation.__name__ == "linear"):
            return False, "dense_1"
        if not (isinstance(model.loss, losses.SparseCategoricalCrossentropy) and model.loss.from_logits):
            return False, "loss"
        if type(model.optimizer) is not optimizers.SGD:
            return False, "optimizer"
        if len(model.trainable_weights) != len(SHAPES):
            return False, "frozen layer weights"
        for m in model.compiled_metrics:
            if m.name not in ("accuracy", "acc", "sparse_categorical_accuracy"):
                return False, f"metric {m.name}"
        return True, ""

    def __init__(self, model, strategy, per_replica_batch, global_batch, exclude=()):
        super().__init__(model, strategy, per_replica_batch, global_batch)
        from ..native import require_C

        C = require_C()
        dev = self.device
        B = per_replica_batch
        self.PP = env.get_int("DAMD_PP", 3)
        if not 1 <= self.PP <= 4:
            raise ValueError("DAMD_PP must be in [1, 4]")
        self.PPB = env.get_int("DAMD_PP_BWD", 2)
        if not 1 <= self.PPB <= 4:
            raise ValueError("DAMD_PP_BWD must be in [1, 4]")
        NS = C.convnet_num_slices(self.PP)
        f32 = dict(dtype=torch.float32, device=dev)
        BP = (B + 63) // 64 * 64
        self.P = torch.zeros(NGRAD, **f32)
        self.G = torch.zeros(C.convnet_grad_count(self.PP), **f32)
        self.V = torch.zeros(NGRAD, **f32)
        self.ctrl = torch.zeros(32, dtype=torch.int32, device=dev)
        self.w1alt = torch.zeros(FEAT * HID, **f32)
        self.v1alt = torch.zeros(FEAT * HID, **f32)
        self.w1bf = torch.zeros(FEAT * HID, dtype=torch.bfloat16, device=dev)
        self.pooled = torch.zeros(FEAT, BP, dtype=torch.bfloat16, device=dev)
        self.code = torch.zeros(B, FEAT, dtype=torch.uint8, device=dev)
        self.hacc = torch.zeros(C.convnet_hacc_elems(B), dtype=torch.int64, device=dev)
        self.hconv = torch.zeros(2 * NCONV, dtype=torch.int64, device=dev)
        self.calt = torch.zeros(2 * NCONV, **f32)
        self.xnext = self.xtag = self.xcur = self.ycur = None
        if B <= 64 and env.get_bool("DAMD_XPREFETCH", True):
            self.xnext = torch.zeros(B * 784, **f32)
            self.xtag = torch.zeros(1, dtype=torch.int64, device=dev)
            self.xcur = torch.zeros(B * 784, **f32)
            self.ycur = torch.zeros(B, dtype=torch.int32, device=dev)
        self.vars = model.trainable_weights
        off = 0
        for v, shp in zip(self.vars, SHAPES):
            if tuple(v.shape) != shp:
                raise RuntimeError(f"unexpected variable shape {v.shape} for {v.name}")
            n = int(np.prod(shp))
            v._rebind(self.P[off:off + n].view(shp))
            off += n
        self._own_variables(self.vars)
        opt = model.optimizer
        if opt.momentum and "momentum" in opt.slots and opt.slots["momentum"].numel() == NPARAM:
            self.V[:NPARAM].copy_(opt.slots["momentum"].to(dev))
        if self.world > 1:
            strategy.communicator.broadcast_(self.P, 0)
        c = self.ctrl.cpu()
        c[C_IT] = int(opt.iterations)
        self.ctrl.copy_(c.to(dev))
        self._write_hparams()
        torch.cuda.synchronize(dev)
        bufs = dict(params=self.P.data_ptr(), grads=self.G.data_ptr(), velocity=self.V.data_ptr(),
                    ctrl=self.ctrl.data_ptr(),
                    pooled=self.pooled.data_ptr(), code=self.code.data_ptr(), w1alt=self.w1alt.data_ptr(),
                    v1alt=self.v1alt.data_ptr(), w1bf=self.w1bf.data_ptr(),
                    hacc=self.hacc.data_ptr(), hconv=self.hconv.data_ptr(), calt=self.calt.data_ptr(),
                    ppb=self.PPB)
        if self.xnext is not None:
            bufs.update(xnext=self.xnext.data_ptr(), xtag=self.xtag.data_ptr(), xcur=self.xcur.data_ptr(),
                        ycur=self.ycur.data_ptr())
        force_ar = env.get_bool("DAMD_FORCE_ALLREDUCE", False)
        self.eager_w1 = self.world == 1 and not force_ar and B <= 64 and env.get_bool("DAMD_EAGER_W1", True)
        bufs["eager_w1"] = int(self.eager_w1)
        bufs["specialised"] = int(env.get_bool("DAMD_SPECIALISED", True))
        self.stamps = None
        if env.get_bool("DAMD_STAMPS", False):
            self.stamps = torch.zeros(3, 256, 16, dtype=torch.int64, device=dev)
            bufs["stamps"] = self.stamps.data_ptr()
        self.trainer = C.ConvNetTrainer(dev.index or 0, bufs, B, self.PP, 1)
        self._refresh_w1bf()
        force = env.get_bool("DAMD_FORCE_ALLREDUCE", False)
        native = strategy.communicator.native if (self.world > 1 or force) else None
        if "rccl" in (exclude or ()):
            native = None
        self.peer = None
        self.sharded = False
        self.exclude = set(exclude or ())
        self.transport_us: dict = {}
        self.exchange_verified = None
        self.exchange_fallback_from: list = []
        self.hred = torch.zeros(2 * NCONV, dtype=torch.int64, device=dev)
        mode = env.get_str("DAMD_ALLREDUCE", "auto").lower()
        self._mode = mode
        if mode not in ("auto", "sharded", "xgmi", "rccl", "off"):
            raise ValueError("DAMD_ALLREDUCE must be auto, sharded, xgmi, rccl or off")
        self.grad_dtype = env.get_str("DAMD_GRAD_DTYPE", "fp32").lower()
        if self.grad_dtype not in ("fp32", "bf16"):
            raise ValueError("DAMD_GRAD_DTYPE must be fp32 or bf16")
        if self.world > 1 and mode not in ("rccl", "off") and not {"xgmi-sharded", "xgmi-peer"} <= self.exclude:
            from ..parallel.communicator import make_peer_allreduce

            from ..utils.watchdog import deadline_for

            wd = deadline_for(self.world)
            want_sharded = mode in ("auto", "sharded") and self.world <= 8
            if want_sharded:
                NU = 4 * C.convnet_num_slices(self.PPB)
                cap = max(self.world * NU * 2048, 347648 + 2 * 8 * 1408 + 16384 + FEAT * HID // 2)
            else:
                cap = C.PeerAllreduce.message_words(C.convnet_grad_count(self.PP), 2 * NCONV)
            self.peer = make_peer_allreduce(strategy.communicator, dev.index or 0, cap,
                                            blocks=env.get_int("DAMD_PEER_BLOCKS", 64),
                                            timeout_s=wd if wd > 0 else 60.0)
            if self.peer is None and mode in ("xgmi", "sharded"):
                raise RuntimeError(f"DAMD_ALLREDUCE={mode} but the xGMI peer mapping is unavailable")
            if self.peer is not None:
                ndev = max(1, torch.cuda.device_count())
                share = [q for q in range(self.world) if q % ndev == (dev.index or 0)]
                cu_split = ((share.index(self.rank), len(share))
                            if len(share) > 2 and env.get_bool("DAMD_SHARED_CU_SPLIT", True) else None)
                cands = [k for k in ((["xgmi-sharded"] if want_sharded else [])
                                     + ([] if mode == "sharded" else ["xgmi-peer"])) if k not in self.exclude]
                tune = (mode == "auto" and env.get_bool("DAMD_XCHG_TUNE", True))
                from . import xchg_selftest

                passed = []
                selftested = env.get_bool("DAMD_XCHG_SELFTEST", True)
                if selftested:
                    for kind in cands:
                        if xchg_selftest.verify(kind, C, strategy.communicator, self.peer, dev, B, self.PPB, self.PP,
                                                self.P, gbf16=self.grad_dtype == "bf16" and kind == "xgmi-sharded",
                                                cu_split=cu_split):
                            passed.append(kind)
                            if not tune:
                                break
                        else:
                            self.exchange_fallback_from.append(kind)
                else:
                    passed = list(cands) if tune else cands[:1]
                chosen = passed[0] if passed else None
                timed = passed + (["rccl"] if (native is not None and "rccl" not in self.exclude) else [])
                if tune and len(timed) > 1:
                    for kind in timed:
                        t = xchg_selftest.time_transport(kind, C, strategy.communicator, self.peer, native, dev, B,
                                                         self.PPB, self.PP, self.P,
                                                         gbf16=self.grad_dtype == "bf16" and kind == "xgmi-sharded",
                                                         cu_split=cu_split)
                        if t is not None:
                            self.transport_us[kind] = round(t * 1e6, 2)
                    if self.transport_us:
                        chosen = min(self.transport_us, key=self.transport_us.get)
                self.peer.set_timeout(env.get_float("DAMD_XCHG_TIMEOUT_S", wd if wd > 0 else 60.0))
                if selftested and chosen is not None and chosen != "rccl":
                    self.exchange_verified = True
                if chosen == "rccl":
                    self.peer = None
                elif chosen is None:
                    if mode in ("xgmi", "sharded"):
                        raise ExchangeSelfTestError(f"DAMD_ALLREDUCE={mode}: the exchange failed its start-up self-test")
                    dlog.warning("fused ConvNet engine: no xGMI exchange passed its self-test; using %s",
                                 "RCCL" if native is not None else "the host (gloo) all-reduce")
                    self.peer = None
                elif chosen == "xgmi-sharded":
                    self.trainer.set_sharded(self.peer, self.hred.data_ptr(), int(self.grad_dtype == "bf16"))
                    self.sharded = True
                    if cu_split is not None:
                        self.trainer.restrict_cus(*cu_split)
                    strategy.communicator.barrier()
        if self.grad_dtype == "bf16" and not self.sharded:
            if self.world > 1:
                dlog.warning("DAMD_GRAD_DTYPE=bf16 applies to the sharded exchange only; exchanging fp32")
            self.grad_dtype = "fp32"
        self.host_collective = self.world > 1 and native is None and self.peer is None
        self.allreduce_kind = ("none" if self.world == 1 and not force else
                               "xgmi-sharded" if self.sharded else
                               "xgmi-peer" if self.peer is not None else
                               "rccl" if native is not None else "host-gloo")
        if self.peer is not None and not self.sharded:
            self.trainer.set_peer(self.peer, fold=env.get_bool("DAMD_PEER_FOLD", True))
        elif self.peer is None and native is not None:
            self.trainer.set_comm(native)
        if self.world > 1:
            dlog.info("fused ConvNet engine: gradient exchange via %s",
                      {"xgmi-sharded": "the step kernels (sharded xGMI exchange)",
                       "xgmi-peer": "xGMI peer-to-peer all-reduce kernel", "rccl": "RCCL",
                       "host-gloo": "host (gloo)"}[self.allreduce_kind])
            if self.transport_us:
                dlog.info("gradient exchange: %s (%s)", self.allreduce_kind,
                          ", ".join(f"{k} {v:.1f} us" for k, v in self.transport_us.items()))
        self.use_graph = env.get_bool("DAMD_GRAPH", True) and not self.host_collective
        self.graph_steps = max(1, env.get_int("DAMD_GRAPH_STEPS", 20))
        self.watchdog_s = env.get_float("DAMD_WATCHDOG_S", 0.0)
        opt._iter_source = self._iterations
        self.feed = None
        self._pending = False
        self.steps_done = 0
        self._fault_done = bool(exclude)
        dlog.debug("fused ConvNet engine: B=%d, slices=%d, graph=%s", B, NS, self.use_graph)

    @property
    def step_kernels(self) -> str:
        return self.trainer.step_kernels

    def _ctrl_host(self, soft=False):
        self.trainer.sync(self.watchdog_s) or self._watchdog_fired()
        self._check_peer(soft)
        return self.ctrl.cpu().tolist()

    def _check_peer(self, soft=False):
        if self.peer is not None and self.peer.status():
            if soft:
                if not getattr(self, "_fault_logged", False):
                    dlog.warning("gradient exchange %s: a bounded wait expired on rank %d; the epoch will be "
                                 "re-run on another transport", self.allreduce_kind, self.rank)
                    self._fault_logged = True
                return
            raise RuntimeError("xGMI peer all-reduce: a wait for a peer timed out (peer missing or wedged)")

    def _ctrl_write(self, updates: dict):
        self.trainer.sync(self.watchdog_s) or self._watchdog_fired()
        self._check_peer()
        c = self.ctrl.cpu()
        for k, v in updates.items():
            c[k] = v
        c[C_XGEN] = (int(c[C_XGEN]) + 1) & 0x7fffffff
        self.ctrl.copy_(c.to(self.device))
        torch.cuda.synchronize(self.device)

    def _write_hparams(self):
        opt = self.model.optimizer
        c = self.ctrl.cpu()
        c[C_LR] = _f2i(opt.learning_rate)
        c[C_MOM] = _f2i(opt.momentum)
        c[C_NEST] = int(opt.nesterov)
        c[C_ROW0] = self.rank * self.per_replica
        c[C_GB] = self.global_batch
        self.ctrl.copy_(c.to(self.device))

    def _watchdog_fired(self):
        what = ("xGMI peer all-reduce wedged" if self.peer is not None else "RCCL communicator aborted")
        raise RuntimeError(f"collective watchdog: step did not complete within {self.watchdog_s}s; {what}")

    def _iterations(self):
        return self._ctrl_host()[C_IT]

    def reload_optimizer_state(self):
        self._flush()
        self.trainer.sync(0.0)
        opt = self.model.optimizer
        if opt.momentum and "momentum" in opt.slots and opt.slots["momentum"].numel() == NPARAM:
            self.V[:NPARAM].copy_(opt.slots["momentum"].to(self.device))
        opt._iter_source = None
        it = int(opt.iterations)
        opt._iter_source = self._iterations
        self._ctrl_write({C_IT: it})

    def lr_changed(self):
        self._flush()
        c = {C_LR: _f2i(self.model.optimizer.learning_rate)}
        self._ctrl_write(c)

    def bind(self, x, y):
        x = np.asarray(x)
        if tuple(x.shape[1:]) not in ((28, 28, 1), (28, 28), (784,)):
            raise ValueError(f"fused ConvNet engine expects 28x28x1 inputs, got {x.shape[1:]}")
        key = (id(x), id(y), len(x))
        if self.feed is None or getattr(self, "_feed_key", None) != key:
            self.trainer.sync(0.0)
            self.feed = DataFeed(x, y, self.device, flatten=True, allow_u8=env.get_bool("DAMD_X_U8", True))
            if self.feed.n * 784 * (1 if self.feed.x_u8 else 4) >= 2 ** 31:
                raise ValueError(f"fused ConvNet engine: {self.feed.n} rows exceed the 2 GiB dataset limit")
            self._feed_key = key
            torch.cuda.synchronize(self.device)
            self.x_ep = torch.empty_like(self.feed.x)
            self.y_ep = torch.empty_like(self.feed.y)
            torch.cuda.synchronize(self.device)
            self.trainer.set_data(self.x_ep.data_ptr(), self.y_ep.data_ptr(), int(self.feed.x_u8))
            self._ctrl_write({C_NS: self.feed.n})
        return self.feed

    def start_epoch(self, epoch, shuffle, wrap_steps: int = 0):
        self._flush()
        self.trainer.sync(0.0)
        self.feed.set_epoch(epoch, shuffle, self.shuffle_seed)
        perm = self.feed.perm.long()
        torch.index_select(self.feed.x, 0, perm, out=self.x_ep)
        torch.index_select(self.feed.y, 0, perm, out=self.y_ep)
        opt = self.model.optimizer
        self._ctrl_write({C_CUR: 0, C_AL: 0, C_AC: 0, C_AN: 0, C_WRAP: int(wrap_steps),
                          C_LR: _f2i(opt.learning_rate), C_MOM: _f2i(opt.momentum), C_NEST: int(opt.nesterov)})

    def run(self, n_steps):
        fa = _xchg_fault_at(self.rank, self.world)
        if fa is not None and self.steps_done <= fa < self.steps_done + n_steps and not self._fault_done:
            import time

            self._fault_done = True
            k = fa - self.steps_done
            if k:
                self.run(k)
            self.trainer.sync(0.0)
            time.sleep(env.get_float("DAMD_XCHG_FAULT_DELAY_S", 3.0))
            self.run(n_steps - k)
            return
        if self.host_collective:
            for _ in range(n_steps):
                self.trainer.step(1)
                self.trainer.sync(0.0)
                self.strategy.communicator.allreduce_(self.G, "sum")
                self.strategy.communicator.allreduce_(self.hconv, "sum")
                torch.cuda.synchronize(self.device)
            self._pending = True
            self.steps_done += n_steps
            return
        if self.use_graph and n_steps >= self.graph_steps:
            self.trainer.capture(self.graph_steps)
        if self.use_graph:
            self.trainer.run(n_steps)
        else:
            self.trainer.step(n_steps)
        self._pending = True
        self.steps_done += n_steps

    def phase_times(self, n_steps: int) -> dict:
        if self.host_collective:
            return super().phase_times(n_steps)
        self.sync()
        rows = self.trainer.phase_times(int(n_steps))
        self._pending = True
        self.steps_done += n_steps
        n = max(len(rows), 1)
        fwd = sum(r[0] for r in rows) / n
        bwd = sum(r[1] for r in rows) / n
        ar = sum(r[2] for r in rows) / n
        return {"forward": fwd, "backward": bwd, "allreduce": ar, "optimizer": 0.0,
                "step": fwd + bwd + ar,
                "note": ("W1 SGD update in the backward kernel, conv / b1 / W2 / b2 updates in the forward kernel"
                         if self.eager_w1 else "SGD update fused into the forward kernel"),
                "allreduce_kind": self.allreduce_kind}

    def prepare(self, n_steps):
        if self.use_graph and not self.host_collective and n_steps >= self.graph_steps:
            self.trainer.capture(self.graph_steps)

    def prepare_final(self, n_steps) -> bool:
        if self.host_collective or not self.use_graph or n_steps <= 0:
            return False
        try:
            self.trainer.capture_final(int(n_steps))
            if env.get_bool("DAMD_WARM_FINAL", True):
                self.trainer.warm_final(int(n_steps))
        except RuntimeError as e:
            dlog.warning("final-graph capture unavailable (%s): timed run replays step graphs + flush", e)
            return False
        return True

    def run_and_flush(self, n_steps):
        if (n_steps > 0 and not self.host_collective and self.use_graph
                and self.trainer.run_final(int(n_steps))):
            self._pending = False
            self.steps_done += n_steps
            return
        self.run(n_steps)
        self._flush()

    def _flush(self):
        if self._pending:
            self.trainer.flush()
            self._pending = False

    def metrics(self):
        soft = self.recovers_faults
        c = self._ctrl_host(soft)
        tail = list(self.trainer.metric_tail()) if self._pending else [0.0, 0.0, 0.0]
        self._check_peer(soft)
        loss = _i2f(c[C_AL]) + tail[0]
        corr = _i2f(c[C_AC]) + tail[1]
        cnt = _i2f(c[C_AN]) + tail[2]
        d = max(cnt, 1.0)
        out = {"loss": float("nan") if c[C_BAD] else loss / d, "_count": cnt}
        for m in self.model.compiled_metrics:
            out[m.name] = corr / d
        return out

    def end_epoch(self):
        self._flush()
        if self.recovers_faults:
            self._vote_exchange_health()
        return self.metrics()

    @property
    def recovers_faults(self) -> bool:
        return (self.world > 1 and self.peer is not None and self._mode == "auto"
                and env.get_bool("DAMD_XCHG_RECOVER", True))

    def recovery_snapshot(self):
        if not self.recovers_faults:
            return None
        self._flush()
        self.trainer.sync(self.watchdog_s) or self._watchdog_fired()
        return {"P": self.P[:NPARAM].cpu().clone(), "V": self.V[:NPARAM].cpu().clone(),
                "it": int(self.ctrl.cpu()[C_IT]), "kind": self.allreduce_kind}

    def _vote_exchange_health(self):
        done = bool(self.trainer.sync(self.watchdog_s if self.watchdog_s > 0 else 120.0))
        st = int(self.peer.status()) if self.peer is not None else 0
        votes = self.strategy.communicator.allgather_object((done, st))
        bad = [r for r, (d, q) in enumerate(votes) if not d or q]
        if bad:
            raise ExchangeFault(f"gradient exchange {self.allreduce_kind}: bounded waits expired on rank(s) {bad}")

    def rebuild_after_fault(self, snap):
        failed = snap["kind"]
        self.trainer.sync(5.0)
        if self.peer is not None:
            self.peer.clear_status()
        torch.cuda.synchronize(self.device)
        self.P[:NPARAM].copy_(snap["P"].to(self.device))
        opt = self.model.optimizer
        opt._iter_source = None
        opt.iterations = snap["it"]
        if opt.momentum:
            opt.ensure_slots(NPARAM, self.device)
            opt.slots["momentum"].copy_(snap["V"].to(self.device))
        torch.cuda.synchronize(self.device)
        self.peer = None
        dlog.warning("gradient exchange %s faulted mid-run: re-running the epoch from its start on the next "
                     "transport", failed)
        new = FusedConvNetEngine(self.model, self.strategy, self.per_replica, self.global_batch,
                                 exclude=self.exclude | {failed})
        new.exchange_fallback_from = list(self.exchange_fallback_from) + [f"{failed} (mid-run)"]
        return new

    def finish(self):
        self._flush()
        self.trainer.sync(self.watchdog_s) or self._watchdog_fired()
        self._check_peer()
        opt = self.model.optimizer
        if opt.momentum:
            opt.ensure_slots(NPARAM, self.device)
            opt.slots["momentum"].copy_(self.V[:NPARAM])
        torch.cuda.synchronize(self.device)

    def _refresh_w1bf(self):
        torch.cuda.synchronize(self.device)
        self.w1bf.copy_(self.P[NCONV:NCONV + FEAT * HID])
        torch.cuda.synchronize(self.device)

    def after_external_write(self):
        self._refresh_w1bf()
        self._ctrl_write({C_BAD: 0})

    def _work_stream(self):
        if getattr(self, "_ext_stream", None) is None:
            self._ext_stream = torch.cuda.ExternalStream(self.trainer.stream, device=self.device)
        return self._ext_stream

    def sync(self):
        self._flush()
        self.trainer.sync(self.watchdog_s) or self._watchdog_fired()
        self._check_peer()
```

Before: 3.708 million images/sec.

## Split flagship backward into conv and W1 role blocks with double-buffered bf16 W1

The specialised backward kernel now launches twice as many blocks. One half does the conv/input-gradient work and the other half does the W1/aux gradient work, each with its own LDS layout, so per-block work and LDS footprint shrink. To let the W1 update write a bf16 copy without racing readers, the bf16 W1 shadow is double-buffered by step parity. A flush-time kernel copies the live buffer back to slot 0. This adds launch plumbing and parity bookkeeping, and there is a risk of stale-buffer bugs when no parity hint is given.

```diff
diff --git a/csrc/bindings.cpp b/csrc/bindings.cpp
--- a/csrc/bindings.cpp
+++ b/csrc/bindings.cpp
@@ -40,6 +40,7 @@
     b_.ctrl = P_<Ctrl>(g("ctrl"));
     b_.pooled = P_<uint16_t>(g("pooled")); b_.code = P_<uint8_t>(g("code"));
     b_.W1alt = P_<float>(g("w1alt")); b_.V1alt = P_<float>(g("v1alt")); b_.w1bf = P_<uint16_t>(g("w1bf"));
+    b_.w1bf_alt = bufs.contains("w1bf_alt") ? P_<uint16_t>(g("w1bf_alt")) : nullptr;
     b_.stamps = bufs.contains("stamps") ? P_<unsigned long long>(g("stamps")) : nullptr;
     b_.eager_w1 = bufs.contains("eager_w1") ? (int)g("eager_w1") : 0;
     b_.hacc = P_<long long>(g("hacc"));
@@ -155,6 +156,7 @@
   }
   void flush() {
     gather();
+    b_.par_hint = hint_ ? par_ : -1;
     HIP_CHECK(convnet2_launch_flush(b_, B_, stream_));
     par_ = 0;
   }
@@ -173,6 +175,7 @@
     return n;
   }
   int bwd_threads() const { return convnet2_bwd_threads(b_, B_, PP_); }
+  int bwd_blocks() const { return convnet2_bwd_blocks(b_, B_, PP_); }
   int bwd_compiled_threads() const {
     int n = 0;
     HIP_CHECK(convnet2_bwd_compiled_threads(b_, B_, PP_, &n));
@@ -253,6 +256,9 @@
   m.attr("CONVNET_NCONV") = kConvNetNConv;
   m.def("convnet2_lds_bytes", [](int PP) { return py::make_tuple(convnet2_fwd_lds(PP, 4), convnet2_bwd_lds(PP)); });
   m.def("convnet2_bwd_flag_lds_bytes", [](int PP) { return convnet2_bwd_lds(PP, true); });
+  m.def("convnet2_bwd_role_lds_bytes", &convnet2_bwd_role_lds, py::arg("positions_per_slice"), py::arg("role"));
+  m.def("convnet2_bwd_flag_blocks", &convnet2_bwd_flag_blocks);
+  m.def("convnet2_bwd_flag_split", &convnet2_bwd_flag_split);
   m.def("convnet_num_slices", &convnet_num_slices);
   m.def("convnet_hacc_elems", &convnet_hacc_elems);
   m.def("convnet_grad_count", &convnet_grad_count);
@@ -367,6 +373,7 @@
       .def_property_readonly("fwd_compiled_threads", &ConvNetTrainer::fwd_compiled_threads)
       .def_property_readonly("bwd_threads", &ConvNetTrainer::bwd_threads)
       .def_property_readonly("bwd_compiled_threads", &ConvNetTrainer::bwd_compiled_threads)
+      .def_property_readonly("bwd_blocks", &ConvNetTrainer::bwd_blocks)
       .def_property_readonly("parity", &ConvNetTrainer::parity)
       .def_property_readonly("stream", [](ConvNetTrainer& t) { return reinterpret_cast<uintptr_t>(t.stream()); });
 
diff --git a/csrc/include/convnet.h b/csrc/include/convnet.h
--- a/csrc/include/convnet.h
+++ b/csrc/include/convnet.h
@@ -29,6 +29,7 @@
   int x_u8;
   float* P; float* G; float* V; Ctrl* ctrl;
   float* W1alt; float* V1alt; uint16_t* w1bf;
+  uint16_t* w1bf_alt;
   uint16_t* pooled ; uint8_t* code ;
   unsigned long long* stamps;
   long long* hacc;
@@ -54,6 +55,10 @@
 int convnet_f1_lg(int B);
 size_t convnet2_fwd_lds(int PP, int lg);
 size_t convnet2_bwd_lds(int PP, bool flagship = false);
+size_t convnet2_bwd_role_lds(int PP, int role);
+int convnet2_bwd_flag_blocks();
+int convnet2_bwd_flag_split();
+int convnet2_bwd_blocks(const ConvNetBuffers& b, int B, int PP);
 hipError_t convnet2_launch_step(const ConvNetBuffers& b, int B, int PP, hipStream_t st);
 hipError_t convnet2_launch_fwd(const ConvNetBuffers& b, int B, int PP, hipStream_t st);
 hipError_t convnet2_launch_bwd(const ConvNetBuffers& b, int B, int PP, hipStream_t st);
diff --git a/csrc/kernels/convnet_step2.hip b/csrc/kernels/convnet_step2.hip
--- a/csrc/kernels/convnet_step2.hip
+++ b/csrc/kernels/convnet_step2.hip
@@ -72,12 +72,15 @@
 #ifndef DAMD_BWD_AUX
 #define DAMD_BWD_AUX 1
 #endif
+#ifndef DAMD_BWD_SPLIT
+#define DAMD_BWD_SPLIT 1
+#endif
 struct CfgGeneric {
   static constexpr int PP = 0, LG = 0;
   static constexpr bool B64 = false, EAGER = false, SH = true;
   static constexpr int NT = 512, BAL = 0, STORES = 0;
   static constexpr bool D1REG = false;
-  static constexpr int AUX = 0;
+  static constexpr int AUX = 0, SPLIT = 0;
 };
 struct CfgFlagFwd {
   static constexpr int PP = 3, LG = 4;
@@ -89,8 +92,9 @@
 struct CfgFlagBwd {
   static constexpr int PP = 2, LG = 0;
   static constexpr bool B64 = true, EAGER = true, SH = false;
-  static constexpr int NT = DAMD_BWD_NT, AUX = DAMD_BWD_AUX;
-  static_assert((NT == 512 || NT == 1024) && AUX >= 0 && AUX <= 1, "bwd wave mapping");
+  static constexpr int NT = DAMD_BWD_NT, AUX = DAMD_BWD_AUX, SPLIT = DAMD_BWD_SPLIT;
+  static_assert((NT == 512 || NT == 1024) && AUX >= 0 && AUX <= 1 && SPLIT >= 0 && SPLIT <= 1, "bwd wave mapping");
+  static constexpr int NSC = (convnet::NPOS + PP - 1) / PP, GRID = SPLIT ? 2 * NSC : NSC;
 };
 __host__ __device__ constexpr int aux_split(int NS) {
   const int chunk_aux = (NAUX2 + NS - 1) / NS;
@@ -109,7 +113,8 @@
                                          uint8_t* __restrict__ code, long long* __restrict__ hacc,
                                          long long* __restrict__ hconv, unsigned long long* st, const XArgs& xa,
                                          const long long* __restrict__ xtag, const int* __restrict__ labels,
-                                         void* __restrict__ xcur, int* __restrict__ ycur, int phint) {
+                                         void* __restrict__ xcur, int* __restrict__ ycur, int phint,
+                                         uint16_t* __restrict__ w1bf_alt) {
   constexpr bool SPEC = C::PP > 0;
   static_assert(!SPEC || (C::B64 && C::EAGER && !C::SH && C::LG == 4), "the one constant configuration");
   constexpr int NT = C::NT, NW = NT / 64, NBQ = SPEC ? (C::PP * 32 * HID / 8 + NT - 1) / NT : 2;
@@ -148,13 +153,14 @@
     xt = *xtag;
   }
   uint4 bq[NBQ];
-  if (eager) {
+  auto load_bq = [&](const uint16_t* __restrict__ src) __attribute__((always_inline)) {
 #pragma unroll
     for (int u = 0; u < NBQ; ++u) {
       bq[u] = make_uint4(0u, 0u, 0u, 0u);
-      if (tid + u * NT < n4 / 2) bq[u] = reinterpret_cast<const uint4*>(w1bf + p0 * 32 * HID)[tid + u * NT];
-    }
-  }
+      if (tid + u * NT < n4 / 2) bq[u] = reinterpret_cast<const uint4*>(src + p0 * 32 * HID)[tid + u * NT];
+    }
+  };
+  if (eager && phint >= 0) load_bq(w1bf);
   const int tcl = min(tid, NCONV - 1);
   const float cp0 = P[tcl], cp1 = calt[tcl], cv0 = V[tcl], cv1 = calt[NCONV + tcl];
   const long long cq0 = sh ? 0 : hconv_r[NCONV + tcl], cq1 = sh ? 0 : hconv_r[tcl];
@@ -180,6 +186,8 @@
   const bool pend = c.pending != 0;
   const long row_base = (long)c.cursor * c.global_batch + c.row0 + img0;
   const bool mom = c.momentum != 0.f;
+  uint16_t* w1live = phint < 0 && par ? w1bf_alt : w1bf;
+  if (eager && phint < 0) load_bq(w1live);
 
   const bool xhit = xnext != nullptr && xt == (((long long)c.xgen << 32) | (long long)(unsigned)(c.cursor + 1));
   if (!xhit) x_load<U8>(xst, X, row_base, c.nsamples, SPEC ? IB : B - img0, lg, r0, nrows, xslot);
@@ -210,7 +218,7 @@
   const bool owner = blockIdx.y == 0;
   float4* Wn4 = reinterpret_cast<float4*>(Wnext + p0 * 32 * HID);
   float4* Vn4 = reinterpret_cast<float4*>(Vnext + p0 * 32 * HID);
-  uint2* Wb = reinterpret_cast<uint2*>(w1bf + p0 * 32 * HID);
+  uint2* Wb = reinterpret_cast<uint2*>(w1live + p0 * 32 * HID);
   if (!eager) {
 #pragma unroll
     for (int u = 0; u < 4; ++u) {
@@ -441,9 +449,10 @@
                                            uint8_t* __restrict__ code, long long* __restrict__ hacc,
                                            long long* __restrict__ hconv, unsigned long long* st, const XArgs xa,
                                            const long long* __restrict__ xtag, const int* __restrict__ labels,
-                                           void* __restrict__ xcur, int* __restrict__ ycur, int phint) {
+                                           void* __restrict__ xcur, int* __restrict__ ycur, int phint,
+                                           uint16_t* __restrict__ w1bf_alt) {
   fwd_body<U8, CfgGeneric>(xnext, w1bf, P, V, calt, hconv_r, G, bpp, lge, ctrl, X, W1alt, V1alt, pooled, code, hacc,
-                           hconv, st, xa, xtag, labels, xcur, ycur, phint);
+                           hconv, st, xa, xtag, labels, xcur, ycur, phint, w1bf_alt);
 }
 
 template <bool U8>
@@ -456,9 +465,10 @@
                                                 uint16_t* __restrict__ pooled, uint8_t* __restrict__ code,
                                                 long long* __restrict__ hacc, long long* __restrict__ hconv,
                                                 unsigned long long* st, const int* __restrict__ labels,
-                                                void* __restrict__ xcur, int* __restrict__ ycur, int phint) {
+                                                void* __restrict__ xcur, int* __restrict__ ycur, int phint,
+                                                uint16_t* __restrict__ w1bf_alt) {
   fwd_body<U8, CfgFlagFwd>(xnext, w1bf, P, V, calt, hconv_r, G, 0, 0, ctrl, X, nullptr, nullptr, pooled, code, hacc,
-                           hconv, st, XArgs{}, xtag, labels, xcur, ycur, phint);
+                           hconv, st, XArgs{}, xtag, labels, xcur, ycur, phint, w1bf_alt);
 }
 
 __device__ __forceinline__ void exchange_tail(const XArgs& xa, Ctrl* ctrl, const float* G, const long long* hconv_p,
@@ -568,7 +578,12 @@
   unsigned long long wst_dh = 0, wst_cg = 0;
   stamp(sts, st, 0);
   constexpr int NSC = SPEC ? (NPOS + C::PP - 1) / C::PP : 1;
-  const int s = blockIdx.x, tid = threadIdx.x, NS = SPEC ? NSC : (int)gridDim.x;
+  constexpr bool SPLIT = SPEC && C::SPLIT != 0;
+  const int wrole = SPLIT && (int)blockIdx.x >= NSC ? 1 : 0;
+  const bool rconv = !SPLIT || wrole == 0, rw1 = !SPLIT || wrole == 1;
+  const int s = SPLIT ? (int)blockIdx.x - wrole * NSC : (int)blockIdx.x, tid = threadIdx.x;
+  const int NS = SPEC ? NSC : (int)gridDim.x;
+  const bool blk0 = blockIdx.x == 0;
   const int auxm = SPEC ? aux_split(NSC) : auxm_;
   const int p0 = s * PP, p1 = min(NPOS, p0 + PP), np = p1 - p0, K = np * 32;
   const int KD = PP * 32 + 4;
@@ -578,15 +593,22 @@
   constexpr bool W16 = NT == 1024, AUXD = C::AUX != 0;
   static_assert(SPEC || (NT == 512 && !AUXD), "the generic kernels keep the plain mapping");
   const int RB = AUXD ? HEAD_BYTES + CH * KD * 4 : max(CH * KD * 4, HEAD_BYTES);
-  float* xs = reinterpret_cast<float*>(smem);
-  float* dps = reinterpret_cast<float*>(smem + XS_BYTES + (AUXD ? HEAD_BYTES : 0));
-  uint16_t* pt = reinterpret_cast<uint16_t*>(smem + XS_BYTES + RB);
-  uint16_t* dht = pt + PP * 32 * HP;
-  uint16_t* dhs = dht + 2 * HID * HP;
-  uint16_t* w1s = dhs + 2 * CH * HP;
-  uint8_t* cs = reinterpret_cast<uint8_t*>(w1s + PP * 32 * HP);
-  float* red = reinterpret_cast<float*>(pt);
-  float* hs = reinterpret_cast<float*>(smem + XS_BYTES);
+  static_assert(!SPLIT || (W16 && AUXD), "the roles build on the 16-wave mapping with dps in its own region");
+  const int PTB = PP * 32 * HP * 2, DHTB = 2 * HID * HP * 2, DHSB = 2 * CH * HP * 2, DPSB = CH * KD * 4;
+  const int o_head = SPLIT ? 0 : XS_BYTES, o_xs = SPLIT ? HEAD_BYTES : 0;
+  const int o_dps = SPLIT ? HEAD_BYTES + XS_BYTES : XS_BYTES + (AUXD ? HEAD_BYTES : 0);
+  const int o_pt = SPLIT ? HEAD_BYTES : XS_BYTES + RB, o_dht = o_pt + PTB;
+  const int o_dhs = SPLIT ? o_dps + DPSB : o_dht + DHTB, o_w1s = o_dhs + DHSB, o_cs = o_w1s + PTB;
+  const int o_red = SPLIT ? o_cs + CH * KC : o_pt, o_ared = SPLIT ? o_dht + DHTB : o_dps;
+  float* xs = reinterpret_cast<float*>(smem + o_xs);
+  float* dps = reinterpret_cast<float*>(smem + o_dps);
+  uint16_t* pt = reinterpret_cast<uint16_t*>(smem + o_pt);
+  uint16_t* dht = reinterpret_cast<uint16_t*>(smem + o_dht);
+  uint16_t* dhs = reinterpret_cast<uint16_t*>(smem + o_dhs);
+  uint16_t* w1s = reinterpret_cast<uint16_t*>(smem + o_w1s);
+  uint8_t* cs = reinterpret_cast<uint8_t*>(smem + o_cs);
+  float* red = reinterpret_cast<float*>(smem + o_red);
+  float* hs = reinterpret_cast<float*>(smem + o_head);
   float* spl = hs + CH * HPITCH;
   float* zs = spl + 716;
   float* rl = zs + CH * ZP;
@@ -601,11 +623,11 @@
   const int chunk_aux = auxm & 0xffff, ltpe = auxm >> 16, tpe = 1 << ltpe;
   const int ae_local = tid >> ltpe, aq = tid & (tpe - 1);
   const int ae = s * chunk_aux + ae_local;
-  const bool aux_on = ae_local < chunk_aux && ae < NAUX2;
+  const bool aux_on = rw1 && ae_local < chunk_aux && ae < NAUX2;
   const int aec = min(ae, NAUX2 - 1);
   float arsum = 0.f;
 
-  const float ag_old = sh ? 0.f : Gr[OFF_LOSS + max(0, min(aec - NSMALL, 2))];
+  const float ag_old = sh || !rw1 ? 0.f : Gr[OFF_LOSS + max(0, min(aec - NSMALL, 2))];
   float spv0 = 0.f, spv1 = 0.f;
   if (!W16 || tid < NSMALL) spv0 = P[OFF_B1 + tid];
   if (!W16 && tid + 512 < NSMALL) spv1 = P[OFF_B1 + tid + 512];
@@ -631,14 +653,19 @@
   constexpr int WS = W16 ? 256 : 512;
   const int wt = W16 ? tid - 768 : tid;
   wv0 = wv1 = make_uint4(0u, 0u, 0u, 0u);
-  if (wt >= 0 && wt < n8) wv0 = reinterpret_cast<const uint4*>(w1bf + p0 * 32 * HID)[wt];
-  if ((!SPEC || WS < PP * 32 * HID / 8) && wt >= 0 && wt + WS < n8)
-    wv1 = reinterpret_cast<const uint4*>(w1bf + p0 * 32 * HID)[wt + WS];
+  auto load_wv = [&](const uint16_t* src) __attribute__((always_inline)) {
+    if (!rconv) return;
+    if (wt >= 0 && wt < n8) wv0 = reinterpret_cast<const uint4*>(src + p0 * 32 * HID)[wt];
+    if ((!SPEC || WS < PP * 32 * HID / 8) && wt >= 0 && wt + WS < n8)
+      wv1 = reinterpret_cast<const uint4*>(src + p0 * 32 * HID)[wt + WS];
+  };
+  if (phint >= 0) load_wv(w1bf);
   constexpr int NB = W16 ? 512 : ONE ? 256 : 512;
   const int bt = ONE ? tid - 256 : tid;
   const bool bw = !ONE || (bt >= 0 && bt < NB);
   const int ct = W16 ? tid - 768 : bt;
-  const bool cw = W16 ? ct >= 0 : bw;
+  const bool bwp = bw && rw1, bwx = bw && rconv;
+  const bool cw = (W16 ? ct >= 0 : bw) && rconv;
   XStage<U8> xst, xst1;
   uint4 pv0, pv1, pv2, pv3;
   uint4 cv, cv1;
@@ -670,7 +697,7 @@
     if (i < CH * kc) v = *reinterpret_cast<const uint4*>(code + (__umul24(min(lb, B - 1), FEAT) + p0 * NF + q * 16));
   };
   auto load_indep = [&](int chunk) __attribute__((always_inline)) {
-    if (bw) {
+    if (bwp) {
       load_pv(pv0, bt, chunk);
       if (NPV > 1) load_pv(pv1, bt + NB, chunk);
       if (ONE && NPV > 2) {
@@ -686,7 +713,7 @@
       const int b = chunk * CH + min(tid, CH - 1);
       ylab = ycur[min(b, B - 1)];
       yval = tid < CH && b < B && ylab >= 0;
-      if (bw) {
+      if (bwx) {
         x_load<U8>(xst, xcur, chunk * CH, B, B - chunk * CH, LG_CH, r0, nrows, bt);
         if (ONE && !W16) x_load<U8>(xst1, xcur, chunk * CH, B, B - chunk * CH, LG_CH, r0, nrows, bt + NB);
       }
@@ -697,10 +724,16 @@
 
   const Ctrl c = *ctrl;
   const int cur = c.cur2, par = phint >= 0 ? phint : c.par2;
-  if (phint >= 0 && phint != c.par2 && s == 0 && tid == 0)
+  if (phint >= 0 && phint != c.par2 && blk0 && tid == 0)
     __hip_atomic_fetch_or(&ctrl->bad, 2, __ATOMIC_RELAXED, __HIP_MEMORY_SCOPE_AGENT);
+  if (phint < 0 && par) {
+    const uint16_t* live = w1bf_out;
+    w1bf_out = const_cast<uint16_t*>(w1bf);
+    w1bf = live;
+  }
+  if (phint < 0) load_wv(w1bf);
   const unsigned xe = (unsigned)c.xcnt2 + 1u;
-  if (s == 0 && tid == 0) {
+  if (blk0 && tid == 0) {
     ctrl->cursor = next_cursor(c, cur);
     ctrl->iterations = c.iterations + 1;
     ctrl->wpar = c.wpar ^ 1;
@@ -714,7 +747,7 @@
   const int ncur = next_cursor(c, cur);
   constexpr int UPI = U8 ? NPIX / 16 : NPIX / 4;
   const int xpu = s * 512 + tid;
-  const bool xpf = ONE && xnext != nullptr && (!W16 || tid < 512) && xpu < B * UPI;
+  const bool xpf = ONE && rw1 && xnext != nullptr && (!W16 || tid < 512) && xpu < B * UPI;
   uint4 xnv = make_uint4(0u, 0u, 0u, 0u);
 
   auto load_dep = [&](int chunk) __attribute__((always_inline)) {
@@ -726,7 +759,7 @@
         yval = tid < CH && b < B && g < c.nsamples;
         ylab = labels[max(0L, min(g, (long)c.nsamples - 1))];
       }
-      if (bw) {
+      if (bwx) {
         x_load<U8>(xst, X, row_base + chunk * CH, c.nsamples, B - chunk * CH, LG_CH, r0, nrows, bt);
         if (ONE && !W16) x_load<U8>(xst1, X, row_base + chunk * CH, c.nsamples, B - chunk * CH, LG_CH, r0, nrows, bt + NB);
       }
@@ -760,15 +793,18 @@
       store_cv(cv, cok, ct);
       if (ONE && !W16 && (!SPEC || NB < CH * KCM)) store_cv(cv1, cok1, ct + NB);
     }
-    if (!bw) return;
-    store_pv(pv0, bt);
-    if (NPV > 1) store_pv(pv1, bt + NB);
-    if (ONE && NPV > 2) {
-      store_pv(pv2, bt + 2 * NB);
-      store_pv(pv3, bt + 3 * NB);
-    }
-    x_store<U8>(xst, xs, LG_CH, nrows);
-    if (ONE && !W16) x_store<U8>(xst1, xs, LG_CH, nrows);
+    if (bwp) {
+      store_pv(pv0, bt);
+      if (NPV > 1) store_pv(pv1, bt + NB);
+      if (ONE && NPV > 2) {
+        store_pv(pv2, bt + 2 * NB);
+        store_pv(pv3, bt + 3 * NB);
+      }
+    }
+    if (bwx) {
+      x_store<U8>(xst, xs, LG_CH, nrows);
+      if (ONE && !W16) x_store<U8>(xst1, xs, LG_CH, nrows);
+    }
   };
   auto store_chunk = [&](int chunk) __attribute__((always_inline)) {
     store_body();
@@ -782,8 +818,8 @@
       xnv = reinterpret_cast<const uint4*>(static_cast<const char*>(X) + __umul24((unsigned)g, U8 ? NPIX : 4 * NPIX))[q];
   }
   const int n8s = SPEC ? PP * 32 * HID / 8 : n8;
-  if (wt >= 0 && wt < n8s) *reinterpret_cast<uint4*>(w1s + (wt >> 3) * HP + (wt & 7) * 8) = wv0;
-  if (wt >= 0 && wt + WS < n8s) *reinterpret_cast<uint4*>(w1s + ((wt + WS) >> 3) * HP + (wt & 7) * 8) = wv1;
+  if (rconv && wt >= 0 && wt < n8s) *reinterpret_cast<uint4*>(w1s + (wt >> 3) * HP + (wt & 7) * 8) = wv0;
+  if (rconv && wt >= 0 && wt + WS < n8s) *reinterpret_cast<uint4*>(w1s + ((wt + WS) >> 3) * HP + (wt & 7) * 8) = wv1;
 
   constexpr int TPW = W16 ? 1 : MAXPP;
   const int dn = wave & 3, dm0 = wave >> 2;
@@ -844,7 +880,7 @@
     else store_chunk(chunk);
     lds_barrier();
     stamp(sts, st, 1);
-    if (ONE && eager) {
+    if (ONE && eager && rw1) {
 #pragma unroll
       for (int i = 0; i < TPW; ++i) {
         const int mt = W16 ? dm0 : dm0 + 2 * i, pi = W16 ? dm0 >> 1 : i;
@@ -958,14 +994,18 @@
         dsum += d;
         hi[j] = f2bf(d);
         lo[j] = bf16_lo(d, hi[j]);
-        dhs[(rb + j) * HP + n] = hi[j];
-        dhs[CH * HP + (rb + j) * HP + n] = lo[j];
-      }
-      *reinterpret_cast<uint2*>(dht + n * HP + rb) =
-          make_uint2((uint32_t)hi[0] | ((uint32_t)hi[1] << 16), (uint32_t)hi[2] | ((uint32_t)hi[3] << 16));
-      *reinterpret_cast<uint2*>(dht + HID * HP + n * HP + rb) =
-          make_uint2((uint32_t)lo[0] | ((uint32_t)lo[1] << 16), (uint32_t)lo[2] | ((uint32_t)lo[3] << 16));
-      db1p[(4 * mt + kq) * HID + n] = dsum;
+        if (rconv) {
+          dhs[(rb + j) * HP + n] = hi[j];
+          dhs[CH * HP + (rb + j) * HP + n] = lo[j];
+        }
+      }
+      if (rw1) {
+        *reinterpret_cast<uint2*>(dht + n * HP + rb) =
+            make_uint2((uint32_t)hi[0] | ((uint32_t)hi[1] << 16), (uint32_t)hi[2] | ((uint32_t)hi[3] << 16));
+        *reinterpret_cast<uint2*>(dht + HID * HP + n * HP + rb) =
+            make_uint2((uint32_t)lo[0] | ((uint32_t)lo[1] << 16), (uint32_t)lo[2] | ((uint32_t)lo[3] << 16));
+        db1p[(4 * mt + kq) * HID + n] = dsum;
+      }
     }
     if (st != nullptr) wst_dh = __builtin_amdgcn_s_memrealtime();
     lds_barrier();
@@ -977,6 +1017,7 @@
     stamp(sts, st, 2);
 #pragma unroll
     for (int i = 0; i < TPW; ++i) {
+      if (!rw1) break;
       const int mt = W16 ? dm0 : dm0 + 2 * i;
       if ((W16 ? dm0 >> 1 : i) >= npl) break;
 #pragma unroll
@@ -989,7 +1030,7 @@
       }
     }
     if (ONE && sh) push_partials();
-    if (ONE && eager) {
+    if (ONE && eager && rw1) {
 #pragma unroll
       for (int i = 0; i < TPW; ++i) {
         const int mt = W16 ? dm0 : dm0 + 2 * i, pi = W16 ? dm0 >> 1 : i;
@@ -1009,7 +1050,8 @@
         }
       }
     }
-    {
+    if (SPLIT && !rconv) stamp(sts, st, 3);
+    if (rconv) {
       const int pm = wave & 3;
 #pragma unroll
       for (int i = 0; i < TPW; ++i) {
@@ -1030,6 +1072,7 @@
     }
     if (C::AUX == 1) aux_sums();
     if (st != nullptr) wst_cg = __builtin_amdgcn_s_memrealtime();
+    if (SPLIT && !rconv) break;
     lds_barrier();
     stamp(sts, st, 3);
     auto conv_grad = [&](auto t0c, auto t1c) __attribute__((always_inline)) {
@@ -1071,15 +1114,17 @@
       G[OFF_W1 + (unsigned)((p0 * 32 + k) * HID + 16 * dn + lr16)] = accw[i][j];
     }
   }
+  if (!SPLIT) lds_barrier();
+  if (rconv) {
+#pragma unroll
+    for (int t = 0; t < 9; ++t)
+      if (!W16 || half == (t >= 5 ? 1 : 0)) red[grp * NCONV + t * NF + ch] = gw[t];
+    if (!W16 || half == 1) red[grp * NCONV + OFF_BC + ch] = gb;
+  }
+  float* ared = reinterpret_cast<float*>(smem + o_ared);
+  if (rw1 && (!W16 || tid < 512)) ared[tid] = arsum;
   lds_barrier();
-#pragma unroll
-  for (int t = 0; t < 9; ++t)
-    if (!W16 || half == (t >= 5 ? 1 : 0)) red[grp * NCONV + t * NF + ch] = gw[t];
-  if (!W16 || half == 1) red[grp * NCONV + OFF_BC + ch] = gb;
-  float* ared = dps;
-  if (!W16 || tid < 512) ared[tid] = arsum;
-  lds_barrier();
-  for (int i = tid; i < (cprobe ? 0 : NCONV); i += NT) {
+  for (int i = tid; i < (cprobe || !rconv ? 0 : NCONV); i += NT) {
     float a = 0.f;
 #pragma unroll
     for (int r = 0; r < 16; ++r) a += red[r * NCONV + i];
@@ -1100,12 +1145,12 @@
   }
   {
     long long* hz = hacc + (long)(par ^ 1) * B * HACC_PITCH;
-    if (!W16 || tid < 512)
+    if (rw1 && (!W16 || tid < 512))
       for (int i = s * 512 + tid; i < B * HID / 2; i += NS * 512)
         *reinterpret_cast<uint4*>(hz + (i >> 5) * HACC_PITCH + (i & 31) * 2) = make_uint4(0u, 0u, 0u, 0u);
   }
   if (xpf) reinterpret_cast<uint4*>(xnext)[xpu] = xnv;
-  if (ONE && xnext != nullptr && s == 0 && tid == 0) *xtag = ((long long)c.xgen << 32) | (long long)(unsigned)(ncur + 1);
+  if (ONE && rw1 && xnext != nullptr && s == 0 && tid == 0) *xtag = ((long long)c.xgen << 32) | (long long)(unsigned)(ncur + 1);
   if (C::SH && sh) exchange_tail(xa, ctrl, G, hconv + par * NCONV, accw, xe, s, NS, np, p0, dn, dm0, lane, tid, xown, xo, xu);
   stamp(sts, st, 5);
   stamp_flush(sts, st, 13);
@@ -1149,8 +1194,10 @@
                                              long long* __restrict__ hconv, const float* __restrict__ calt,
                                              long long* __restrict__ hacc, int B, int eager,
                                              uint16_t* __restrict__ w1bf, Ctrl* __restrict__ ctrl,
-                                             long long* __restrict__ hconv_w) {
+                                             long long* __restrict__ hconv_w, int phint) {
   const Ctrl c = *ctrl;
+  if (phint >= 0 && phint != c.wpar && blockIdx.x == 0 && threadIdx.x == 0)
+    __hip_atomic_fetch_or(&ctrl->bad, 2, __ATOMIC_RELAXED, __HIP_MEMORY_SCOPE_AGENT);
   const bool mom = c.momentum != 0.f, pend = c.pending != 0;
   const long long* hg = hconv + (c.wpar ^ 1) * NCONV;
   const int nvisit = eager ? NPARAM - (OFF_B1 - OFF_W1) : NPARAM;
@@ -1195,6 +1242,13 @@
       ctrl->ticket = 0;
     }
   }
+}
+
+__global__ __launch_bounds__(512) void w1bf_live0(const Ctrl* __restrict__ ctrl, const uint4* __restrict__ b1,
+                                                  uint4* __restrict__ b0) {
+  if (ctrl->wpar == 0) return;
+  const int i = blockIdx.x * 512 + threadIdx.x;
+  if (i < FEAT * HID / 8) b0[i] = b1[i];
 }
 
 __global__ __launch_bounds__(512) void sh_gather(Ctrl* __restrict__ ctrl, const XArgs xa, long long* __restrict__ hred,
@@ -1244,8 +1298,23 @@
   const size_t xsb = (size_t)IB * XR * IMG * 4, partb = (size_t)IB * HID * 4;
   return (xsb > partb ? xsb : partb) + (size_t)(IB + HID) * KP * 2 + CONV_LDS_BYTES + (size_t)IB * PP * 32 + 256 * 4;
 }
+size_t convnet2_bwd_role_lds(int PP, int role) {
+  using namespace convnet;
+  const size_t head = (size_t)convnet2::HEAD_BYTES, tile = (size_t)PP * 32 * HP * 2, slack = 16 + 256 * 4;
+  if (role == 0)
+    return head + XS_BYTES + (size_t)CH * (PP * 32 + 4) * 4 + (size_t)2 * CH * HP * 2 + tile + (size_t)CH * PP * 32 +
+           (size_t)16 * NCONV * 4 + slack;
+  return head + tile + (size_t)2 * HID * HP * 2 + (size_t)512 * 4 + slack;
+}
+int convnet2_bwd_flag_blocks() { return convnet2::CfgFlagBwd::GRID; }
+int convnet2_bwd_flag_split() { return convnet2::CfgFlagBwd::SPLIT; }
+
 size_t convnet2_bwd_lds(int PP, bool flagship) {
   using namespace convnet;
+  if (flagship && convnet2::CfgFlagBwd::SPLIT != 0) {
+    const size_t a = convnet2_bwd_role_lds(PP, 0), b = convnet2_bwd_role_lds(PP, 1);
+    return a > b ? a : b;
+  }
   const int KD = PP * 32 + 4;
   const size_t dpsb = (size_t)CH * KD * 4;
   const size_t rb = flagship && convnet2::CfgFlagBwd::AUX != 0 ? (size_t)convnet2::HEAD_BYTES + dpsb
@@ -1270,8 +1339,19 @@
 bool convnet2_specialised(const ConvNetBuffers& b, int B, int PP) {
   using namespace convnet;
   using namespace convnet2;
+  const bool two = b.w1bf_alt != nullptr && b.w1bf_alt != b.w1bf;
   return !b.force_generic && !b.xa && !b.Gr && !b.hconv_r && B == CH && PP == CfgFlagFwd::PP &&
-         convnet_f1_lg(B) == CfgFlagFwd::LG && ppb_of(b, PP) == CfgFlagBwd::PP && eager2(b, B) == 1;
+         convnet_f1_lg(B) == CfgFlagFwd::LG && ppb_of(b, PP) == CfgFlagBwd::PP && eager2(b, B) == 1 &&
+         (two || CfgFlagBwd::SPLIT == 0);
+}
+
+struct W1bfPair {
+  uint16_t* live;
+  uint16_t* other;
+};
+static W1bfPair w1bf_pair(const ConvNetBuffers& b) {
+  uint16_t* alt = b.w1bf_alt ? b.w1bf_alt : b.w1bf;
+  return b.par_hint == 1 ? W1bfPair{alt, b.w1bf} : W1bfPair{b.w1bf, alt};
 }
 
 template <bool U8>
@@ -1280,17 +1360,18 @@
   const int NS = convnet_num_slices(PP);
   const int lg = convnet_f1_lg(B);
   const dim3 g1(NS, (B + (1 << lg) - 1) >> lg);
+  const W1bfPair w1 = w1bf_pair(b);
   if (convnet2_specialised(b, B, PP)) {
     hipLaunchKernelGGL((convnet2::fwd_flag<U8>), g1, dim3(convnet2::CfgFlagFwd::NT), convnet2_fwd_lds(PP, lg), st,
-                       b.xnext, b.xtag, b.w1bf, b.P, b.V, b.calt, b.hconv, b.G, b.ctrl, b.X, b.pooled, b.code, b.hacc,
-                       b.hconv, b.stamps, b.labels, b.xcur, b.ycur, b.par_hint);
+                       b.xnext, b.xtag, w1.live, b.P, b.V, b.calt, b.hconv, b.G, b.ctrl, b.X, b.pooled, b.code, b.hacc,
+                       b.hconv, b.stamps, b.labels, b.xcur, b.ycur, b.par_hint, w1.other);
     return;
   }
   hipLaunchKernelGGL((convnet2::fwd<U8>), g1, dim3(512), convnet2_fwd_lds(PP, lg), st,
-                     B <= CH ? b.xnext : nullptr, b.w1bf, b.P, b.V, b.calt, b.hconv_r ? b.hconv_r : b.hconv,
+                     B <= CH ? b.xnext : nullptr, w1.live, b.P, b.V, b.calt, b.hconv_r ? b.hconv_r : b.hconv,
                      b.Gr ? b.Gr : b.G, B | (PP << 16), lg | (eager2(b, B) << 8), b.ctrl, b.X, b.W1alt, b.V1alt,
                      b.pooled, b.code, b.hacc, b.hconv, b.stamps, xargs(b), b.xtag, b.labels,
-                     B <= CH ? b.xcur : nullptr, b.ycur, b.par_hint);
+                     B <= CH ? b.xcur : nullptr, b.ycur, b.par_hint, w1.other);
 }
 
 template <bool U8>
@@ -1299,20 +1380,21 @@
   const int PP = ppb_of(b, PPf);
   const int NS = convnet_num_slices(PP);
   const int auxm = convnet2::aux_split(NS);
+  const W1bfPair w1 = w1bf_pair(b);
   if (convnet2_specialised(b, B, PPf))
-    hipLaunchKernelGGL((convnet2::bwd_flag<U8>), dim3(NS), dim3(convnet2::CfgFlagBwd::NT), convnet2_bwd_lds(PP, true), st, b.hacc, b.ycur, b.xcur,
-                       b.P, b.w1bf, b.pooled, b.code, b.par_hint, b.G, b.ctrl, b.X, b.labels, b.G, b.hconv, b.P, b.V,
-                       b.w1bf, b.stamps ? b.stamps + 2 * 256 * 16 : nullptr, b.xnext, b.xtag);
+    hipLaunchKernelGGL((convnet2::bwd_flag<U8>), dim3(convnet2::CfgFlagBwd::GRID), dim3(convnet2::CfgFlagBwd::NT), convnet2_bwd_lds(PP, true), st, b.hacc, b.ycur, b.xcur,
+                       b.P, w1.live, b.pooled, b.code, b.par_hint, b.G, b.ctrl, b.X, b.labels, b.G, b.hconv, b.P, b.V,
+                       w1.other, b.stamps ? b.stamps + 2 * 256 * 16 : nullptr, b.xnext, b.xtag);
   else if (B <= CH)
     hipLaunchKernelGGL((convnet2::bwd<U8, true>), dim3(NS), dim3(512), convnet2_bwd_lds(PP), st, b.hacc,
                        B <= CH ? b.ycur : nullptr, B <= CH ? b.xcur : nullptr, b.par_hint, B | (PP << 16), b.P,
-                       b.w1bf, b.pooled, b.code, b.ctrl, b.X, b.labels, b.G, b.hconv, eager2(b, B), b.P, b.V, b.w1bf,
+                       w1.live, b.pooled, b.code, b.ctrl, b.X, b.labels, b.G, b.hconv, eager2(b, B), b.P, b.V, w1.other,
                        b.stamps ? b.stamps + 2 * 256 * 16 : nullptr, b.Gr ? b.Gr : b.G, xargs(b), b.xnext, b.xtag,
                        auxm);
   else
     hipLaunchKernelGGL((convnet2::bwd<U8, false>), dim3(NS), dim3(512), convnet2_bwd_lds(PP), st, b.hacc,
                        B <= CH ? b.ycur : nullptr, B <= CH ? b.xcur : nullptr, b.par_hint, B | (PP << 16), b.P,
-                       b.w1bf, b.pooled, b.code, b.ctrl, b.X, b.labels, b.G, b.hconv, eager2(b, B), b.P, b.V, b.w1bf,
+                       w1.live, b.pooled, b.code, b.ctrl, b.X, b.labels, b.G, b.hconv, eager2(b, B), b.P, b.V, w1.other,
                        b.stamps ? b.stamps + 2 * 256 * 16 : nullptr, b.Gr ? b.Gr : b.G, xargs(b), b.xnext, b.xtag,
                        auxm);
 }
@@ -1329,6 +1411,10 @@
   const hipError_t e = hipFuncGetAttributes(&at, f);
   if (e == hipSuccess) *out = at.maxThreadsPerBlock;
   return e;
+}
+
+int convnet2_bwd_blocks(const ConvNetBuffers& b, int B, int PP) {
+  return convnet2_specialised(b, B, PP) ? convnet2::CfgFlagBwd::GRID : convnet_num_slices(ppb_of(b, PP));
 }
 
 int convnet2_bwd_threads(const ConvNetBuffers& b, int B, int PP) {
@@ -1377,9 +1463,12 @@
 }
 
 hipError_t convnet2_launch_flush(const ConvNetBuffers& b, int B, hipStream_t st) {
+  if (eager2(b, B) && b.w1bf_alt && b.w1bf_alt != b.w1bf && b.par_hint != 0)
+    hipLaunchKernelGGL(convnet2::w1bf_live0, dim3((convnet::FEAT * convnet::HID / 8 + 511) / 512), dim3(512), 0, st, b.ctrl,
+                       reinterpret_cast<const uint4*>(b.w1bf_alt), reinterpret_cast<uint4*>(b.w1bf));
   hipLaunchKernelGGL(convnet2::flush, dim3(eager2(b, B) ? 1 : 340), dim3(eager2(b, B) ? 1024 : 256), 0, st, b.P, b.Gr ? b.Gr : b.G, b.V,
                      b.W1alt, b.V1alt, b.hconv_r ? b.hconv_r : b.hconv, b.calt, b.hacc, B, eager2(b, B), b.w1bf, b.ctrl,
-                     b.hconv);
+                     b.hconv, b.par_hint);
   return hipGetLastError();
 }
 
diff --git a/distributed_amd/engine/fused_convnet.py b/distributed_amd/engine/fused_convnet.py
--- a/distributed_amd/engine/fused_convnet.py
+++ b/distributed_amd/engine/fused_convnet.py
@@ -106,7 +106,7 @@
         self.ctrl = torch.zeros(32, dtype=torch.int32, device=dev)
         self.w1alt = torch.zeros(FEAT * HID, **f32)
         self.v1alt = torch.zeros(FEAT * HID, **f32)
-        self.w1bf = torch.zeros(FEAT * HID, dtype=torch.bfloat16, device=dev)
+        self.w1bf_bufs = tuple(torch.zeros(FEAT * HID, dtype=torch.bfloat16, device=dev) for _ in range(2))
         self.pooled = torch.zeros(FEAT, BP, dtype=torch.bfloat16, device=dev)
         self.code = torch.zeros(B, FEAT, dtype=torch.uint8, device=dev)
         self.hacc = torch.zeros(C.convnet_hacc_elems(B), dtype=torch.int64, device=dev)
@@ -140,7 +140,8 @@
         bufs = dict(params=self.P.data_ptr(), grads=self.G.data_ptr(), velocity=self.V.data_ptr(),
                     ctrl=self.ctrl.data_ptr(),
                     pooled=self.pooled.data_ptr(), code=self.code.data_ptr(), w1alt=self.w1alt.data_ptr(),
-                    v1alt=self.v1alt.data_ptr(), w1bf=self.w1bf.data_ptr(),
+                    v1alt=self.v1alt.data_ptr(), w1bf=self.w1bf_bufs[0].data_ptr(),
+                    w1bf_alt=self.w1bf_bufs[1].data_ptr(),
                     hacc=self.hacc.data_ptr(), hconv=self.hconv.data_ptr(), calt=self.calt.data_ptr(),
                     ppb=self.PPB)
         if self.xnext is not None:
@@ -519,9 +520,14 @@
             opt.slots["momentum"].copy_(self.V[:NPARAM])
         torch.cuda.synchronize(self.device)
 
+    @property
+    def w1bf(self):
+        return self.w1bf_bufs[self.trainer.parity]
+
     def _refresh_w1bf(self):
         torch.cuda.synchronize(self.device)
-        self.w1bf.copy_(self.P[NCONV:NCONV + FEAT * HID])
+        for buf in self.w1bf_bufs:
+            buf.copy_(self.P[NCONV:NCONV + FEAT * HID])
         torch.cuda.synchronize(self.device)
 
     def after_external_write(self):
```

New measurement: 3.805 million images/sec, median of 6. 2.6% higher.
